# buaacyw/MeshAnything

Measured on NVIDIA H100. Metric: face-tokens/sec (350M, 800-face cap), higher is better.
Workload: dtype f16 weights/activations, f32 accumulate

## Files before the change

include/meshanything_b200.h:

```cpp
#ifndef MESHANYTHING_B200_H
#define MESHANYTHING_B200_H

#include <stddef.h>
#include <stdint.h>

#ifdef __cplusplus
extern "C" {
#endif

#define MA_ABI_VERSION 1
#define MA_MAX_LAYERS 32

#define MA_EPI_NONE 0
#define MA_EPI_RELU 1
#define MA_EPI_GELU 2
#define MA_LIN_SEG64 0x10
#define MA_LIN_SEG256 0x20

int ma_abi_version(void);
const char* ma_last_error(void);


int ma_linear_f16(const void* W, const void* bias, const void* x, int ldx, void* y, int ldy, int M, int N, int K,
                  int epilogue, void* stream);

int ma_layernorm(const float* x, const void* res16, const float* gamma, const float* beta, float eps, int M, int W,
                 float* out32, void* out16, void* stream);

size_t ma_attention_scratch_bytes(int M, int H, int max_keys);
int ma_attention_f16(const void* q, int ldq, const void* K, const void* V, long T, int H, const int* slots,
                     const int* nkeys, int max_keys, int M, float scale, void* out, int ldo, void* scratch,
                     void* stream);
int ma_attention_decode_f16(const void* qkv, int ldq, void* K, void* V, long T, const int* nkeys, int max_keys, int M,
                            float scale, void* out, int ldo, void* scratch, void* stream);


typedef struct {
  int n_layers, vocab, codebook, npos;
  const void* wqkv[MA_MAX_LAYERS];
  const void* bqkv[MA_MAX_LAYERS];
  const void* wo[MA_MAX_LAYERS];
  const void* bo[MA_MAX_LAYERS];
  const void* w1[MA_MAX_LAYERS];
  const void* b1[MA_MAX_LAYERS];
  const void* w2[MA_MAX_LAYERS];
  const void* b2[MA_MAX_LAYERS];
  const float* ln1g[MA_MAX_LAYERS];
  const float* ln1b[MA_MAX_LAYERS];
  const float* ln2g[MA_MAX_LAYERS];
  const float* ln2b[MA_MAX_LAYERS];
  const void* lm_head;
  const void* tok_table;
  const float* extra;
  const float* tok_pos;
  const float* cond;
  const float* pos;
} ma_decoder_weights;

typedef struct {
  int do_sample;
  int top_k;
  float top_p;
  uint64_t seed;
} ma_sampling;

int ma_sample_tokens(const void* logits, int B, int vocab, const ma_sampling* sampling, int32_t* out_tokens,
                     int32_t* out_support, void* stream);

size_t ma_kv_cache_bytes(int n_layers, int B, int tmax);
size_t ma_decoder_workspace_bytes(int B, int tmax);

int ma_decode_generate(const ma_decoder_weights* w, const float* prefix, int B, int tmax, int max_new,
                       const ma_sampling* sampling, int eos_id, int pad_id, void* kv, void* ws, int32_t* out_ids,
                       int32_t* out_lens, const int32_t* forced_ids, void* logits_out, int flags, void* stream);

int ma_decode_slots_init(int B, int tmax, int pad_id, void* ws, void* stream);
int ma_decode_slot_stream(int slot, int B, int tmax, int stream_id, void* ws, void* stream);
int ma_decode_slots_seek(int B, int tmax, int pos, int gen, int tok, void* ws, void* stream);
int ma_decode_slot_prefill(const ma_decoder_weights* w, const float* prefix, int slot, int B, int tmax, int max_new,
                           const ma_sampling* sampling, int eos_id, int pad_id, void* kv, void* ws, int32_t* out_ids,
                           void* stream);
int ma_decode_slots_step(const ma_decoder_weights* w, int B, int tmax, int max_new, int n_steps, int max_ctx,
                         const ma_sampling* sampling, int eos_id, int pad_id, void* kv, void* ws, int32_t* out_ids,
                         int flags, void* stream);
int ma_decode_slots_poll(int B, int tmax, void* ws, int32_t* finished_host, int32_t* lens_host, void* stream);

#define MA_GEN_NO_GRAPH 1
#define MA_GEN_NO_FAST 2
#define MA_GEN_NO_PDL 4
#define MA_GEN_NO_EARLY_EXIT 8
#define MA_GEN_NO_MEGA 16
#define MA_GEN_TC 64
#define MA_GEN_TRACE 32

int ma_decoder_debug(void* ws, int B, int tmax, int what, void* host_out, int nbytes);
void ma_mega_set_debug(unsigned long long timeout_ns, int fault);
int ma_decode_persistent_supported(void);


int ma_linear_tc_f16(const void* W, const void* bias, const void* x, int ldx, void* y, int ldy, int M, int N, int K,
                     int epilogue, void* stream);
size_t ma_linear_ws_scratch_bytes(void);
void ma_linear_ws_set_mode(int cluster);
int ma_linear_ws_f16(const void* W, const void* bias, const void* x, int ldx, void* y, int ldy, int M, int N, int K,
                     int epilogue, void* scratch, void* stream);
int ma_set_tensor_cores(int enable);
void ma_tensor_core_linear_counts(unsigned long long* on_tensor_cores, unsigned long long* canonical_fallback);

int ma_attention_tc_f16(const void* q, int ldq, const void* K, const void* Vt, long T, long Tpad, int H,
                        int rows_per_slot, int n_slots, int nkeys, float scale, void* out, int ldo, void* stream);
int ma_transpose_heads_f16(const void* src, int ld, int col0, int head_stride, int H, int n, long Tpad, int n_slots,
                           void* dst, void* stream);


typedef struct {
  const void* c_qkv_w;
  const void *c_proj_w, *c_proj_b;
  const float *ln1_g, *ln1_b, *ln2_g, *ln2_b;
  const void *fc_w, *fc_b;
  const void *proj_w, *proj_b;
} ma_miche_block;

typedef struct {
  const void *input_proj_w, *input_proj_b;
  const float* query;
  const void *cq_w, *ckv_w;
  const void *cproj_w, *cproj_b;
  const float *ln1_g, *ln1_b, *ln2_g, *ln2_b, *ln3_g, *ln3_b;
  const void *fc_w, *fc_b, *proj_w, *proj_b;
  ma_miche_block enc[8];
  const float *lnpost_g, *lnpost_b;
  const void *pre_kl_w, *pre_kl_b;
  const void *post_kl_w, *post_kl_b;
  ma_miche_block dec[16];
  const void *cond_head_w, *cond_head_b;
  const void *cond_w, *cond_b;
} ma_encoder_weights;

size_t ma_encoder_workspace_bytes(int B);

int ma_encoder_forward(const ma_encoder_weights* w, const void* pc_normal, int B, float* point_feature, float* prefix,
                       void* ws, void* stream);


typedef struct {
  const void *in_w, *in_b;
  const void *out_w, *out_b;
  const void *l1_w, *l1_b;
  const void *l2_w, *l2_b;
  const float *n1_g, *n1_b, *n2_g, *n2_b;
} ma_bert_layer;

typedef struct {
  int n_layers;
  ma_bert_layer layer[8];
  const float* pos_embedding;
  const float* point_pe;
  const float *ln_g, *ln_b, *pln_g, *pln_b;
  const void *cond_w, *cond_b, *cond_head_w, *cond_head_b;
  const void *down_w, *down_b;
  const void *coor_w, *coor_b;
  const float* codebook;
} ma_tokenizer_weights;

size_t ma_detokenize_workspace_bytes(int B, int F);

int ma_detokenize(const ma_tokenizer_weights* w, const int32_t* gen_ids, int max_new, int B, int F,
                  const float* point_feature, float* out_xyz, int32_t* ids_out, void* ws, void* stream);

size_t ma_sample_surface_workspace_bytes(int n_faces);
int ma_sample_surface(const float* vertices, const int32_t* faces, int n_faces, int n_samples, unsigned long long seed,
                      void* out_pc_normal, int32_t* out_face_idx, void* ws, void* stream);

unsigned long long ma_launch_count(void);

#ifdef __cplusplus
}
#endif
#endif
```

meshanything_b200/capi.py:

```python
from __future__ import annotations

import ctypes as C
import os
from typing import Optional

import torch

from . import build as _build

MA_MAX_LAYERS = 32
EPI_NONE, EPI_RELU, EPI_GELU = 0, 1, 2
LIN_SEG64, LIN_SEG256 = 0x10, 0x20
GEN_NO_GRAPH, GEN_NO_FAST, GEN_NO_PDL, GEN_NO_EARLY_EXIT, GEN_NO_MEGA, GEN_TRACE, GEN_TC = 1, 2, 4, 8, 16, 32, 64

_vp = C.c_void_p


class DecoderWeights(C.Structure):
    _fields_ = (
        [("n_layers", C.c_int), ("vocab", C.c_int), ("codebook", C.c_int), ("npos", C.c_int)]
        + [(n, _vp * MA_MAX_LAYERS) for n in ("wqkv", "bqkv", "wo", "bo", "w1", "b1", "w2", "b2",
                                              "ln1g", "ln1b", "ln2g", "ln2b")]
        + [(n, _vp) for n in ("lm_head", "tok_table", "extra", "tok_pos", "cond", "pos")]
    )


class Sampling(C.Structure):
    _fields_ = [("do_sample", C.c_int), ("top_k", C.c_int), ("top_p", C.c_float), ("seed", C.c_uint64)]


_lib = None

EXPORTS = [
    "ma_abi_version", "ma_last_error", "ma_launch_count", "ma_linear_f16", "ma_layernorm",
    "ma_attention_scratch_bytes", "ma_attention_f16", "ma_attention_decode_f16", "ma_kv_cache_bytes", "ma_decoder_workspace_bytes",
    "ma_decode_generate", "ma_decoder_debug", "ma_encoder_workspace_bytes", "ma_encoder_forward",
    "ma_detokenize_workspace_bytes", "ma_detokenize", "ma_linear_tc_f16", "ma_set_tensor_cores", "ma_sample_tokens",
    "ma_attention_tc_f16", "ma_transpose_heads_f16",
    "ma_decode_slots_init", "ma_decode_slot_prefill", "ma_decode_slots_step", "ma_decode_slots_poll",
    "ma_mega_set_debug", "ma_linear_ws_set_mode", "ma_decode_slots_seek", "ma_decode_slot_stream", "ma_linear_ws_scratch_bytes", "ma_linear_ws_f16",
    "ma_sample_surface_workspace_bytes", "ma_sample_surface", "ma_tensor_core_linear_counts", "ma_decode_persistent_supported",
]


def lib_path() -> str:
    return _build.LIB


def lib():
    global _lib
    if _lib is not None:
        return _lib
    path = _build.LIB
    dev_tree = os.path.isdir(os.path.join(os.path.dirname(os.path.dirname(os.path.abspath(__file__))), ".git"))
    stale = (os.path.exists(path) and dev_tree and _build.have_nvcc()
             and os.environ.get("MA_B200_NO_AUTOBUILD") != "1" and _build._stale())
    if not os.path.exists(path) or stale or (os.environ.get("MA_B200_REBUILD") == "1"):
        path = _build.build(force=True)
    L = C.CDLL(path)
    L.ma_abi_version.restype = C.c_int
    L.ma_last_error.restype = C.c_char_p
    L.ma_launch_count.restype = C.c_ulonglong
    L.ma_linear_f16.argtypes = [_vp, _vp, _vp, C.c_int, _vp, C.c_int, C.c_int, C.c_int, C.c_int, C.c_int, _vp]
    L.ma_layernorm.argtypes = [_vp, _vp, _vp, _vp, C.c_float, C.c_int, C.c_int, _vp, _vp, _vp]
    L.ma_attention_scratch_bytes.argtypes = [C.c_int, C.c_int, C.c_int]
    L.ma_attention_scratch_bytes.restype = C.c_size_t
    L.ma_attention_f16.argtypes = [_vp, C.c_int, _vp, _vp, C.c_long, C.c_int, _vp, _vp, C.c_int, C.c_int,
                                   C.c_float, _vp, C.c_int, _vp, _vp]
    L.ma_kv_cache_bytes.argtypes = [C.c_int, C.c_int, C.c_int]
    L.ma_kv_cache_bytes.restype = C.c_size_t
    L.ma_decoder_workspace_bytes.argtypes = [C.c_int, C.c_int]
    L.ma_decoder_workspace_bytes.restype = C.c_size_t
    L.ma_decode_generate.argtypes = [C.POINTER(DecoderWeights), _vp, C.c_int, C.c_int, C.c_int, C.POINTER(Sampling),
                                     C.c_int, C.c_int, _vp, _vp, _vp, _vp, _vp, _vp, C.c_int, _vp]
    L.ma_sample_tokens.argtypes = [_vp, C.c_int, C.c_int, C.POINTER(Sampling), _vp, _vp, _vp]
    L.ma_attention_decode_f16.argtypes = [_vp, C.c_int, _vp, _vp, C.c_long, _vp, C.c_int, C.c_int, C.c_float, _vp, C.c_int,
                                          _vp, _vp]
    L.ma_attention_tc_f16.argtypes = [_vp, C.c_int, _vp, _vp, C.c_long, C.c_long, C.c_int, C.c_int, C.c_int, C.c_int,
                                      C.c_float, _vp, C.c_int, _vp]
    L.ma_transpose_heads_f16.argtypes = [_vp, C.c_int, C.c_int, C.c_int, C.c_int, C.c_int, C.c_long, C.c_int, _vp, _vp]
    L.ma_decode_slots_init.argtypes = [C.c_int, C.c_int, C.c_int, _vp, _vp]
    L.ma_linear_ws_set_mode.argtypes = [C.c_int]
    L.ma_linear_ws_set_mode.restype = None
    L.ma_decode_slot_stream.argtypes = [C.c_int, C.c_int, C.c_int, C.c_int, _vp, _vp]
    L.ma_decode_slots_seek.argtypes = [C.c_int, C.c_int, C.c_int, C.c_int, C.c_int, _vp, _vp]
    L.ma_decode_slot_prefill.argtypes = [C.POINTER(DecoderWeights), _vp, C.c_int, C.c_int, C.c_int, C.c_int,
                                         C.POINTER(Sampling), C.c_int, C.c_int, _vp, _vp, _vp, _vp]
    L.ma_decode_slots_step.argtypes = [C.POINTER(DecoderWeights), C.c_int, C.c_int, C.c_int, C.c_int, C.c_int,
                                       C.POINTER(Sampling), C.c_int, C.c_int, _vp, _vp, _vp, C.c_int, _vp]
    L.ma_decode_slots_poll.argtypes = [C.c_int, C.c_int, _vp, _vp, _vp, _vp]
    L.ma_decoder_debug.argtypes = [_vp, C.c_int, C.c_int, C.c_int, _vp, C.c_int]
    L.ma_mega_set_debug.argtypes = [C.c_ulonglong, C.c_int]
    L.ma_mega_set_debug.restype = None
    L.ma_decode_persistent_supported.argtypes = []
    L.ma_decode_persistent_supported.restype = C.c_int
    L.ma_encoder_workspace_bytes.argtypes = [C.c_int]
    L.ma_encoder_workspace_bytes.restype = C.c_size_t
    L.ma_encoder_forward.argtypes = [_vp, _vp, C.c_int, _vp, _vp, _vp, _vp]
    L.ma_detokenize_workspace_bytes.argtypes = [C.c_int, C.c_int]
    L.ma_detokenize_workspace_bytes.restype = C.c_size_t
    L.ma_detokenize.argtypes = [_vp, _vp, C.c_int, C.c_int, C.c_int, _vp, _vp, _vp, _vp, _vp]
    L.ma_linear_ws_scratch_bytes.restype = C.c_size_t
    L.ma_linear_ws_f16.argtypes = [_vp, _vp, _vp, C.c_int, _vp, C.c_int, C.c_int, C.c_int, C.c_int, C.c_int, _vp, _vp]
    L.ma_sample_surface_workspace_bytes.argtypes = [C.c_int]
    L.ma_sample_surface_workspace_bytes.restype = C.c_size_t
    L.ma_sample_surface.argtypes = [_vp, _vp, C.c_int, C.c_int, C.c_ulonglong, _vp, _vp, _vp, _vp]
    L.ma_linear_tc_f16.argtypes = [_vp, _vp, _vp, C.c_int, _vp, C.c_int, C.c_int, C.c_int, C.c_int, C.c_int, _vp]
    L.ma_set_tensor_cores.argtypes = [C.c_int]
    L.ma_tensor_core_linear_counts.argtypes = [C.POINTER(C.c_ulonglong), C.POINTER(C.c_ulonglong)]
    L.ma_tensor_core_linear_counts.restype = None
    if L.ma_abi_version() != 1:
        raise RuntimeError("libmeshanything_b200.so: ABI version mismatch")
    _lib = L
    return L


def check(rc: int, what: str):
    if rc != 0:
        raise RuntimeError(f"{what} failed: {lib().ma_last_error().decode()}")


def ptr(t: Optional[torch.Tensor]):
    return None if t is None else C.c_void_p(t.data_ptr())


def stream_ptr() -> C.c_void_p:
    return C.c_void_p(torch.cuda.current_stream().cuda_stream)


def _need_cuda(*ts):
    for t in ts:
        if t is not None and not t.is_cuda:
            raise RuntimeError("meshanything_b200: tensors must live on a CUDA device (no CPU fallback)")



def linear_f16(w: torch.Tensor, bias: Optional[torch.Tensor], x: torch.Tensor, epilogue: int = EPI_NONE,
               out: Optional[torch.Tensor] = None) -> torch.Tensor:
    _need_cuda(w, bias, x)
    assert w.dtype == torch.float16 and x.dtype == torch.float16 and w.is_contiguous()
    assert x.dim() == 2 and x.stride(1) == 1
    M, K = x.shape
    N = w.shape[0]
    if out is None:
        out = torch.empty((M, N), dtype=torch.float16, device=x.device)
    check(lib().ma_linear_f16(ptr(w), ptr(bias), ptr(x), x.stride(0), ptr(out), out.stride(0), M, N, K, epilogue,
                              stream_ptr()), "ma_linear_f16")
    return out


def sample_surface(vertices: torch.Tensor, faces: torch.Tensor, n_samples: int, seed: int = 0,
                   want_index: bool = False):
    _need_cuda(vertices, faces)
    v = vertices.to(torch.float32).contiguous()
    f = faces.to(torch.int32).contiguous()
    F = f.shape[0]
    ws = torch.empty(lib().ma_sample_surface_workspace_bytes(F), dtype=torch.uint8, device=v.device)
    out = torch.empty((n_samples, 6), dtype=torch.float16, device=v.device)
    idx = torch.empty((n_samples,), dtype=torch.int32, device=v.device) if want_index else None
    check(lib().ma_sample_surface(ptr(v), ptr(f), F, n_samples, int(seed), ptr(out), ptr(idx), ptr(ws), stream_ptr()),
          "ma_sample_surface")
    return (out, idx) if want_index else out


def tensor_core_linear_counts():
    a, b = C.c_ulonglong(0), C.c_ulonglong(0)
    lib().ma_tensor_core_linear_counts(C.byref(a), C.byref(b))
    return a.value, b.value


_ws_scratch = {}


def linear_ws_f16(w: torch.Tensor, bias: Optional[torch.Tensor], x: torch.Tensor, epilogue: int = EPI_NONE) -> torch.Tensor:
    _need_cuda(w, bias, x)
    M, K = x.shape
    N = w.shape[0]
    scr = _ws_scratch.get(x.device)
    if scr is None:
        scr = _ws_scratch[x.device] = torch.zeros(lib().ma_linear_ws_scratch_bytes(), dtype=torch.uint8, device=x.device)
    out = torch.empty((M, N), dtype=torch.float16, device=x.device)
    check(lib().ma_linear_ws_f16(ptr(w), ptr(bias), ptr(x), x.stride(0), ptr(out), out.stride(0), M, N, K, epilogue,
                                 ptr(scr), stream_ptr()), "ma_linear_ws_f16")
    return out


def linear_tc_f16(w: torch.Tensor, bias: Optional[torch.Tensor], x: torch.Tensor, epilogue: int = EPI_NONE) -> torch.Tensor:
    _need_cuda(w, bias, x)
    M, K = x.shape
    N = w.shape[0]
    out = torch.empty((M, N), dtype=torch.float16, device=x.device)
    check(lib().ma_linear_tc_f16(ptr(w), ptr(bias), ptr(x), x.stride(0), ptr(out), out.stride(0), M, N, K, epilogue,
                                 stream_ptr()), "ma_linear_tc_f16")
    return out


def transpose_heads_f16(src: torch.Tensor, col0: int, head_stride: int, H: int, n: int, n_slots: int) -> torch.Tensor:
    _need_cuda(src)
    Tpad = (n + 127) // 128 * 128
    dst = torch.empty((n_slots, H, 64, Tpad), dtype=torch.float16, device=src.device)
    check(lib().ma_transpose_heads_f16(ptr(src), src.stride(0), col0, head_stride, H, n, Tpad, n_slots, ptr(dst),
                                       stream_ptr()), "ma_transpose_heads_f16")
    return dst


def attention_tc_f16(q: torch.Tensor, k: torch.Tensor, vt: torch.Tensor, nkeys: int, rows_per_slot: int,
                     scale: float = 0.125) -> torch.Tensor:
    _need_cuda(q, k, vt)
    S, H, T, _ = k.shape
    Tpad = vt.shape[3]
    assert q.is_contiguous() and k.is_contiguous() and vt.is_contiguous() and q.shape[0] == S * rows_per_slot
    out = torch.empty_like(q)
    check(lib().ma_attention_tc_f16(ptr(q), q.stride(0), ptr(k), ptr(vt), T, Tpad, H, rows_per_slot, S, nkeys,
                                    C.c_float(scale), ptr(out), out.stride(0), stream_ptr()), "ma_attention_tc_f16")
    return out


def sample_tokens(logits: torch.Tensor, do_sample: bool = True, top_k: int = 50, top_p: float = 0.95, seed: int = 0,
                  want_support: bool = False):
    _need_cuda(logits)
    assert logits.dtype == torch.float16 and logits.is_contiguous()
    B, vocab = logits.shape
    tok = torch.empty((B,), dtype=torch.int32, device=logits.device)
    sup = torch.empty((B, 256), dtype=torch.int32, device=logits.device) if want_support else None
    s = Sampling(int(do_sample), int(top_k), float(top_p), int(seed))
    check(lib().ma_sample_tokens(ptr(logits), B, vocab, C.byref(s), ptr(tok), ptr(sup), stream_ptr()),
          "ma_sample_tokens")
    return (tok, sup) if want_support else tok


def layernorm(x: Optional[torch.Tensor], res16: Optional[torch.Tensor], gamma: torch.Tensor, beta: torch.Tensor,
              eps: float = 1e-5, want32: bool = True, want16: bool = True):
    _need_cuda(x, res16, gamma, beta)
    src = x if x is not None else res16
    M, W = src.shape
    o32 = torch.empty((M, W), dtype=torch.float32, device=src.device) if want32 else None
    o16 = torch.empty((M, W), dtype=torch.float16, device=src.device) if want16 else None
    check(lib().ma_layernorm(ptr(x), ptr(res16), ptr(gamma), ptr(beta), eps, M, W, ptr(o32), ptr(o16), stream_ptr()),
          "ma_layernorm")
    return o32, o16


def attention_decode_f16(qkv: torch.Tensor, k: torch.Tensor, v: torch.Tensor, nkeys: torch.Tensor,
                         scale: float = 0.125) -> torch.Tensor:
    _need_cuda(qkv, k, v, nkeys)
    M = qkv.shape[0]
    assert qkv.shape[1] == 3072 and qkv.is_contiguous() and k.is_contiguous() and v.is_contiguous()
    assert k.shape[0] == M and k.shape[1] == 16 and k.shape[3] == 64
    T = k.shape[2]
    max_keys = int(nkeys.max().item())
    scratch = torch.zeros(lib().ma_attention_scratch_bytes(M, 16, max_keys), dtype=torch.uint8, device=qkv.device)
    out = torch.empty((M, 1024), dtype=torch.float16, device=qkv.device)
    check(lib().ma_attention_decode_f16(ptr(qkv), 3072, ptr(k), ptr(v), T, ptr(nkeys), max_keys, M, scale, ptr(out),
                                        1024, ptr(scratch), stream_ptr()), "ma_attention_decode_f16")
    return out


def attention_f16(q: torch.Tensor, k: torch.Tensor, v: torch.Tensor, nkeys: torch.Tensor,
                  slots: Optional[torch.Tensor] = None, scale: float = 0.125) -> torch.Tensor:
    _need_cuda(q, k, v, nkeys, slots)
    M, H, D = q.shape
    assert D == 64 and k.is_contiguous() and v.is_contiguous() and q.is_contiguous()
    T = k.shape[2]
    max_keys = int(nkeys.max().item())
    scratch = torch.zeros(lib().ma_attention_scratch_bytes(M, H, max_keys), dtype=torch.uint8, device=q.device)
    out = torch.empty((M, H, D), dtype=torch.float16, device=q.device)
    check(lib().ma_attention_f16(ptr(q), H * D, ptr(k), ptr(v), T, H, ptr(slots), ptr(nkeys), max_keys, M, scale,
                                 ptr(out), H * D, ptr(scratch), stream_ptr()), "ma_attention_f16")
    return out
```

meshanything_b200/csrc/api.cu:

```cuda
#include <stdarg.h>
#include <stdlib.h>
#include <stdio.h>
#include <string.h>

#include <atomic>
#include <map>
#include <mutex>
#include <vector>

#include "canon.cuh"
#include "internal.h"

namespace ma {

static thread_local char g_err[512] = "";
static std::atomic<unsigned long long> g_launches{0};

void set_error(const char* fmt, ...) {
  va_list ap;
  va_start(ap, fmt);
  vsnprintf(g_err, sizeof(g_err), fmt, ap);
  va_end(ap);
}
void count_launch(int n) { g_launches += (unsigned long long)n; }
bool check_launch(const char* what) {
  cudaError_t e = cudaPeekAtLastError();
  if (e != cudaSuccess) {
    set_error("%s: %s", what, cudaGetErrorString(e));
    cudaGetLastError();
    return false;
  }
  return true;
}

static inline size_t align_up(size_t x, size_t a = 256) { return (x + a - 1) / a * a; }

constexpr int PREFILL_SEQS = 8;

struct DecWs {
  float* hres;
  __half *x16, *qkv, *attn16, *y16, *f16, *logits, *lastx16;
  int* nkeys;
  SeqState s;
  int* all_done;
  void* attn_scratch;
  size_t attn_scratch_bytes;
  void* attn_scratch_pre;
  size_t attn_scratch_pre_bytes;
  void* fast;
  void* mega;
  void* tc_scratch;
  size_t total;
};

static DecWs carve(void* base, int B, int tmax, int vocab) {
  DecWs w;
  const size_t rows = (size_t)std::max(B, PREFIX * std::min(B, PREFILL_SEQS));
  size_t off = 0;
  auto take = [&](size_t bytes) {
    void* p = base ? (void*)((char*)base + off) : nullptr;
    off += align_up(bytes);
    return p;
  };
  w.hres = (float*)take(rows * HID * 4);
  w.x16 = (__half*)take(rows * HID * 2);
  w.qkv = (__half*)take(rows * QKV * 2);
  w.attn16 = (__half*)take(rows * HID * 2);
  w.y16 = (__half*)take(rows * HID * 2);
  w.f16 = (__half*)take(rows * FFN * 2);
  w.logits = (__half*)take((size_t)B * vocab * 2);
  w.lastx16 = (__half*)take((size_t)B * HID * 2);
  w.nkeys = (int*)take(rows * 4);
  w.s.pos = (int*)take((size_t)B * 4);
  w.s.gen = (int*)take((size_t)B * 4);
  w.s.tok = (int*)take((size_t)B * 4);
  w.s.finished = (int*)take((size_t)B * 4);
  w.s.lens = (int*)take((size_t)B * 4);
  w.s.sid = (int*)take((size_t)B * 4);
  w.all_done = (int*)take(256);
  w.attn_scratch_bytes = attention_scratch_bytes((int)B, NHEAD, tmax);
  w.attn_scratch = take(w.attn_scratch_bytes);
  w.attn_scratch_pre_bytes = attention_scratch_bytes(PREFIX * std::min(B, PREFILL_SEQS), NHEAD, PREFIX);
  w.attn_scratch_pre = take(w.attn_scratch_pre_bytes);
  w.fast = take(fast_workspace_bytes());
  w.mega = take(mega_workspace_bytes());
  w.tc_scratch = take(linear_ws_scratch_bytes());
  w.total = off;
  return w;
}

static inline __half* kv_layer(void* kv, int layer, int which, int B, long T) {
  return (__half*)kv + ((size_t)(layer * 2 + which) * B) * NHEAD * T * HD;
}

static const bool g_no_stream_attn = [] {
  const char* e = getenv("MA_B200_NO_STREAM_ATTN");
  return e && e[0] == '1';
}();

static const bool g_no_pdl = [] {
  const char* e = getenv("MA_B200_NO_PDL");
  return e && e[0] == '1';
}();

static int dec_linear(bool tc, const DecWs& ws, const void* W, const void* b, const __half* x, int ldx, __half* y, int ldy,
                      int M, int N, int K, int epi, cudaStream_t st, bool pdl = false) {
  if (tc) {
    const bool tiled_ok = M >= 64 && linear_tc_supported(M, N, K, ldx, ldy, x, W, y);
    const bool ws_ok = M <= 128 && linear_ws_supported(M, N, K, ldx, x, W);
    if (ws_ok && (linear_ws_mode() || !tiled_ok || K > 1024))
      return launch_linear_ws((const __half*)W, (const __half*)b, x, ldx, y, ldy, M, N, K, epi, ws.tc_scratch, st, pdl);
    if (tiled_ok) return launch_linear_tc((const __half*)W, (const __half*)b, x, ldx, y, ldy, M, N, K, epi, st);
  }
  return launch_linear((const __half*)W, (const __half*)b, x, ldx, y, ldy, M, N, K, epi, st);
}

static int run_layers(const ma_decoder_weights* w, const DecWs& ws, void* kv, int B, long T, int M, int rows_per_slot,
                      int slot0, int max_keys, cudaStream_t st, bool tc = false) {
  void* scratch = rows_per_slot > 1 ? ws.attn_scratch_pre : ws.attn_scratch;
  const bool pdl = tc && rows_per_slot == 1 && !g_no_pdl;
  for (int L = 0; L < w->n_layers; L++) {
    __half* kc = kv_layer(kv, L, 0, B, T) + (size_t)slot0 * NHEAD * T * HD;
    __half* vc = kv_layer(kv, L, 1, B, T) + (size_t)slot0 * NHEAD * T * HD;
    if (dec_linear(tc, ws, w->wqkv[L], w->bqkv[L], ws.x16, HID, ws.qkv, QKV, M, QKV, HID, MA_EPI_NONE, st, pdl)) return 1;
    if (rows_per_slot == 1 && !g_no_stream_attn) {
      if (launch_attention_decode(ws.qkv, QKV, kc, vc, T, ws.nkeys, max_keys, M, 0.125f, ws.attn16, HID, scratch, pdl,
                                  st)) return 1;
    } else {
      if (launch_kv_append(ws.qkv, M, rows_per_slot, ws.nkeys, kc, vc, T, st)) return 1;
      if (launch_attention(ws.qkv, QKV, kc, vc, T, NHEAD, rows_per_slot, nullptr, ws.nkeys, max_keys, M, 0.125f,
                           ws.attn16, HID, scratch, st)) return 1;
    }
    if (dec_linear(tc, ws, w->wo[L], w->bo[L], ws.attn16, HID, ws.y16, HID, M, HID, HID, MA_EPI_NONE, st, pdl)) return 1;
    if (launch_layernorm(ws.hres, ws.y16, w->ln1g[L], w->ln1b[L], MA_LN_EPS, M, HID, ws.hres, ws.x16, st, pdl)) return 1;
    if (dec_linear(tc, ws, w->w1[L], w->b1[L], ws.x16, HID, ws.f16, FFN, M, FFN, HID, MA_EPI_RELU, st, pdl)) return 1;
    if (dec_linear(tc, ws, w->w2[L], w->b2[L], ws.f16, FFN, ws.y16, HID, M, HID, FFN, MA_EPI_NONE, st, pdl)) return 1;
    if (launch_layernorm(ws.hres, ws.y16, w->ln2g[L], w->ln2b[L], MA_LN_EPS, M, HID, ws.hres, ws.x16, st, pdl)) return 1;
  }
  return 0;
}

struct GraphKey {
  const void *w, *kv, *ws, *out_ids, *forced, *logits_out;
  unsigned long long whash;
  int B, tmax, max_new, bucket, flags, do_sample, top_k, eos, pad, mode;
  float top_p;
  unsigned long long seed;
  bool operator<(const GraphKey& o) const { return memcmp(this, &o, sizeof(GraphKey)) < 0; }
};
static std::map<GraphKey, cudaGraphExec_t> g_graphs;
static std::map<cudaGraphExec_t, unsigned long long> g_graph_launches;
static cudaStream_t g_stream = nullptr;
static int* g_flag_host = nullptr;
static cudaEvent_t g_ev_in = nullptr, g_ev_out = nullptr, g_ev_flag = nullptr;

static int g_device = -1;
static std::mutex g_mu;

static int ensure_globals() {
  int dev = -1;
  if (cudaGetDevice(&dev) != cudaSuccess) {
    set_error("cudaGetDevice: %s", cudaGetErrorString(cudaGetLastError()));
    return 1;
  }
  if (g_device >= 0 && dev != g_device) {
    set_error("ma_decode_generate was first used on device %d; this process now runs on device %d "
              "(one process per GPU)", g_device, dev);
    return 1;
  }
  if (!g_stream) {
    if (cudaStreamCreateWithFlags(&g_stream, cudaStreamNonBlocking) != cudaSuccess ||
        cudaHostAlloc((void**)&g_flag_host, 64, cudaHostAllocDefault) != cudaSuccess ||
        cudaEventCreateWithFlags(&g_ev_in, cudaEventDisableTiming) != cudaSuccess ||
        cudaEventCreateWithFlags(&g_ev_out, cudaEventDisableTiming) != cudaSuccess ||
        cudaEventCreateWithFlags(&g_ev_flag, cudaEventDisableTiming) != cudaSuccess) {
      set_error("cannot create stream/events: %s", cudaGetErrorString(cudaGetLastError()));
      return 1;
    }
    g_device = dev;
  }
  return 0;
}


static int enqueue_batched_step(const ma_decoder_weights* w, const DecWs& ws, void* kv, int B, long T, int max_keys,
                                const SampleArgs& sa, cudaStream_t s, bool tc) {
  if (launch_embed_tokens(w, ws.s, B, ws.hres, ws.x16, ws.nkeys, s)) return 1;
  if (run_layers(w, ws, kv, B, T, B, 1, 0, max_keys, s, tc)) return 1;
  if (dec_linear(tc, ws, w->lm_head, nullptr, ws.x16, HID, ws.logits, w->vocab, B, w->vocab, HID, MA_EPI_NONE, s,
                 tc && !g_no_pdl)) return 1;
  return launch_sample(sa, s);
}

static inline bool use_tc(int B, int do_sample, int flags) { return B > 1 && (do_sample || (flags & MA_GEN_TC)); }

static unsigned long long weights_hash(const ma_decoder_weights* w) {
  unsigned long long h = 1469598103934665603ull;
  const unsigned char* pb = (const unsigned char*)w;
  for (size_t q = 0; q < sizeof(ma_decoder_weights); q++) h = (h ^ pb[q]) * 1099511628211ull;
  return h;
}

template <class F>
static int launch_cached_graph(const GraphKey& key, cudaStream_t st, F&& enqueue) {
  auto it = g_graphs.find(key);
  if (it == g_graphs.end()) {
    cudaGraph_t graph = nullptr;
    if (cudaStreamBeginCapture(st, cudaStreamCaptureModeThreadLocal) != cudaSuccess) {
      set_error("cudaStreamBeginCapture: %s", cudaGetErrorString(cudaGetLastError()));
      return 1;
    }
    const unsigned long long before = g_launches.load();
    int erc = enqueue(st);
    const unsigned long long per_step = g_launches.load() - before;
    cudaError_t ce = cudaStreamEndCapture(st, &graph);
    if (erc || ce != cudaSuccess || !graph) {
      if (!erc) set_error("cudaStreamEndCapture: %s", cudaGetErrorString(ce));
      cudaGetLastError();
      return 1;
    }
    cudaGraphExec_t exec = nullptr;
    ce = cudaGraphInstantiate(&exec, graph, 0);
    cudaGraphDestroy(graph);
    if (ce != cudaSuccess) {
      set_error("cudaGraphInstantiate: %s", cudaGetErrorString(ce));
      return 1;
    }
    if (g_graphs.size() > 64) {
      for (auto& kvp : g_graphs) cudaGraphExecDestroy(kvp.second);
      g_graphs.clear();
      g_graph_launches.clear();
    }
    it = g_graphs.emplace(key, exec).first;
    g_launches -= per_step;
    g_graph_launches[exec] = per_step;
  }
  if (cudaGraphLaunch(it->second, st) != cudaSuccess) {
    set_error("cudaGraphLaunch: %s", cudaGetErrorString(cudaGetLastError()));
    return 1;
  }
  g_launches += g_graph_launches[it->second];
  return 0;
}

static void fill_sample_args(SampleArgs& sa, const ma_decoder_weights* w, const DecWs& ws, int B, int max_new,
                             const ma_sampling* sampling, int eos_id, int pad_id, int32_t* out_ids) {
  memset(&sa, 0, sizeof(sa));
  sa.logits = ws.logits; sa.vocab = w->vocab; sa.B = B; sa.max_new = max_new; sa.eos_id = eos_id; sa.pad_id = pad_id;
  sa.do_sample = sampling ? sampling->do_sample : 0;
  sa.top_k = sampling ? sampling->top_k : 0;
  sa.top_p = sampling ? sampling->top_p : 1.0f;
  sa.seed = sampling ? sampling->seed : 0;
  sa.s = ws.s; sa.out_ids = out_ids;
}

static int check_decode_args(const char* who, const ma_decoder_weights* w, int B, int tmax, int max_new) {
  if (w->n_layers > MA_MAX_LAYERS || w->vocab > 8195 + 61) {
    set_error("%s: n_layers=%d / vocab=%d unsupported", who, w->n_layers, w->vocab);
    return 1;
  }
  if (B <= 0 || max_new <= 0 || PREFIX + max_new > tmax) {
    set_error("%s: B=%d, tmax=%d < 257 + max_new=%d", who, B, tmax, max_new);
    return 1;
  }
  if (PREFIX + max_new + 2 > w->npos) {
    set_error("%s: sequence of %d exceeds %d learned positions", who, PREFIX + max_new, w->npos - 2);
    return 1;
  }
  return 0;
}

}

using namespace ma;

extern "C" {

int ma_abi_version(void) { return MA_ABI_VERSION; }
const char* ma_last_error(void) { return g_err; }
unsigned long long ma_launch_count(void) { return g_launches.load(); }

int ma_linear_f16(const void* W, const void* bias, const void* x, int ldx, void* y, int ldy, int M, int N, int K,
                  int epilogue, void* stream) {
  return launch_linear((const __half*)W, (const __half*)bias, (const __half*)x, ldx, (__half*)y, ldy, M, N, K,
                       epilogue, (cudaStream_t)stream);
}

size_t ma_linear_ws_scratch_bytes(void) { return linear_ws_scratch_bytes(); }
void ma_linear_ws_set_mode(int cluster) { linear_ws_set_mode(cluster); }

int ma_linear_ws_f16(const void* W, const void* bias, const void* x, int ldx, void* y, int ldy, int M, int N, int K,
                     int epilogue, void* scratch, void* stream) {
  return launch_linear_ws((const __half*)W, (const __half*)bias, (const __half*)x, ldx, (__half*)y, ldy, M, N, K,
                          epilogue, scratch, (cudaStream_t)stream);
}

int ma_layernorm(const float* x, const void* res16, const float* gamma, const float* beta, float eps, int M, int W,
                 float* out32, void* out16, void* stream) {
  return launch_layernorm(x, (const __half*)res16, gamma, beta, eps, M, W, out32, (__half*)out16,
                          (cudaStream_t)stream);
}

size_t ma_attention_scratch_bytes(int M, int H, int max_keys) { return attention_scratch_bytes(M, H, max_keys); }

int ma_attention_f16(const void* q, int ldq, const void* K, const void* V, long T, int H, const int* slots,
                     const int* nkeys, int max_keys, int M, float scale, void* out, int ldo, void* scratch,
                     void* stream) {
  if (M > 65535) {
    set_error("ma_attention_f16: M=%d exceeds 65535 rows per call", M);
    return 1;
  }
  return launch_attention((const __half*)q, ldq, (const __half*)K, (const __half*)V, T, H, 1, slots, nkeys, max_keys, M,
                          scale, (__half*)out, ldo, scratch, (cudaStream_t)stream);
}

int ma_attention_decode_f16(const void* qkv, int ldq, void* K, void* V, long T, const int* nkeys, int max_keys, int M,
                            float scale, void* out, int ldo, void* scratch, void* stream) {
  if (!qkv || !K || !V || !nkeys || !out || !scratch || M < 1 || max_keys < 1 || max_keys > T || ldq < 3 * HID) {
    set_error("ma_attention_decode_f16: bad arguments (M=%d, max_keys=%d, T=%ld, ldq=%d)", M, max_keys, T, ldq);
    return 1;
  }
  return launch_attention_decode((const __half*)qkv, ldq, (__half*)K, (__half*)V, T, nkeys, max_keys, M, scale,
                                 (__half*)out, ldo, scratch, false, (cudaStream_t)stream);
}

int ma_sample_tokens(const void* logits, int B, int vocab, const ma_sampling* sampling, int32_t* out_tokens,
                     int32_t* out_support, void* stream) {
  if (!logits || !out_tokens || B < 1 || vocab < 1) {
    set_error("ma_sample_tokens: bad arguments");
    return 1;
  }
  SampleArgs sa;
  memset(&sa, 0, sizeof(sa));
  sa.logits = (const __half*)logits; sa.vocab = vocab; sa.B = B; sa.max_new = 1; sa.eos_id = -1; sa.pad_id = -1;
  sa.do_sample = sampling ? sampling->do_sample : 0;
  sa.top_k = sampling ? sampling->top_k : 0;
  sa.top_p = sampling ? sampling->top_p : 1.0f;
  sa.seed = sampling ? sampling->seed : 0;
  sa.first = 1; sa.token_out = out_tokens; sa.support_out = out_support;
  return launch_sample(sa, (cudaStream_t)stream);
}

size_t ma_kv_cache_bytes(int n_layers, int B, int tmax) {
  return (size_t)n_layers * 2 * B * NHEAD * (size_t)tmax * HD * sizeof(__half);
}

size_t ma_decoder_workspace_bytes(int B, int tmax) { return carve(nullptr, B, tmax, 8195 + 61).total; }

int ma_decode_generate(const ma_decoder_weights* w, const float* prefix, int B, int tmax, int max_new,
                       const ma_sampling* sampling, int eos_id, int pad_id, void* kv, void* ws_, int32_t* out_ids,
                       int32_t* out_lens, const int32_t* forced_ids, void* logits_out, int flags, void* stream) {
  if (!w || !prefix || !kv || !ws_ || !out_ids || B <= 0 || max_new <= 0) {
    set_error("ma_decode_generate: bad arguments");
    return 1;
  }
  if (check_decode_args("ma_decode_generate", w, B, tmax, max_new)) return 1;
  std::lock_guard<std::mutex> lock(g_mu);
  if (ensure_globals()) return 1;
  cudaStream_t user = (cudaStream_t)stream;
  cudaStream_t st = g_stream;
  cudaEventRecord(g_ev_in, user);
  cudaStreamWaitEvent(st, g_ev_in, 0);

  const long T = tmax;
  DecWs ws = carve(ws_, B, tmax, 8195 + 61);
  cudaMemsetAsync(ws.attn_scratch, 0, ws.attn_scratch_bytes, st);
  cudaMemsetAsync(ws.attn_scratch_pre, 0, ws.attn_scratch_pre_bytes, st);
  cudaMemsetAsync(ws.fast, 0, fast_workspace_bytes(), st);
  if (launch_fill_i32(out_ids, pad_id, (long)B * max_new, st)) return 1;

  SampleArgs sa;
  fill_sample_args(sa, w, ws, B, max_new, sampling, eos_id, pad_id, out_ids);
  sa.first = 1; sa.forced = forced_ids; sa.logits_out = (__half*)logits_out;
  sa.all_done = ws.all_done;

  const bool tc = use_tc(B, sa.do_sample, flags);
  if (tc) cudaMemsetAsync(ws.tc_scratch, 0, linear_ws_scratch_bytes(), st);
  const bool fast = (B == 1) && !(flags & MA_GEN_NO_FAST);
  bool mega = fast && !sa.do_sample && !(flags & MA_GEN_NO_MEGA) && mega_fits(tmax) && mega_supported();
  if (fast) sa.nkeys_next = fast_nkeys_ptr(ws.fast);
  if (mega && mega_prepare(w, ws.mega, st)) mega = false;

  for (int b0 = 0; b0 < B; b0 += PREFILL_SEQS) {
    const int nb = std::min(PREFILL_SEQS, B - b0), M = nb * PREFIX;
    if (launch_embed_prefix(w, prefix + (size_t)b0 * PREFIX * HID, nb, ws.hres, ws.x16, ws.nkeys, st)) return 1;
    if (run_layers(w, ws, kv, B, T, M, PREFIX, b0, PREFIX, st, tc)) return 1;
    if (launch_gather_rows(ws.x16, HID, PREFIX - 1, PREFIX, nb, ws.lastx16 + (size_t)b0 * HID, st)) return 1;
  }
  if (dec_linear(tc, ws, w->lm_head, nullptr, ws.lastx16, HID, ws.logits, w->vocab, B, w->vocab, HID, MA_EPI_NONE, st))
    return 1;
  if (launch_sample(sa, st)) return 1;
  sa.first = 0;
  sa.nkeys_next = nullptr;


  const bool use_graph = !(flags & MA_GEN_NO_GRAPH);
  const bool early = !(flags & MA_GEN_NO_EARLY_EXIT) && !forced_ids;
  const int CHECK_EVERY = 64;
  const unsigned long long whash = use_graph ? weights_hash(w) : 0;
  bool flag_pending = false;
  int rc = 0;
  if (mega) {
    const int MEGA_STEPS = 512;
    for (int i = 1; i < max_new && rc == 0; i += MEGA_STEPS) {
      rc = mega_enqueue(w, ws.s, tmax, (__half*)kv, ws.mega, sa, std::min(MEGA_STEPS, max_new - i), i - 1,
                        (flags & MA_GEN_TRACE) ? 1 : 0, st);
    }
  }
  for (int i = 1; i < max_new && rc == 0 && !mega; i++) {
    const int ctx = PREFIX + i;
    const int bucket = fast ? 0 : (ctx + 1023) / 1024;
    const int max_keys = fast ? tmax : std::min(tmax, bucket * 1024);
    auto enqueue = [&](cudaStream_t s) -> int {
      if (fast) return fast_step_enqueue(w, ws.s, tmax, (__half*)kv, ws.fast, sa, !(flags & MA_GEN_NO_PDL), s);
      return enqueue_batched_step(w, ws, kv, B, T, max_keys, sa, s, tc);
    };
    if (!use_graph) {
      rc = enqueue(st);
    } else {
      GraphKey key;
      memset(&key, 0, sizeof(key));
      key.w = w; key.kv = kv; key.ws = ws_; key.out_ids = out_ids; key.forced = forced_ids; key.logits_out = logits_out;
      key.B = B; key.tmax = tmax; key.max_new = max_new; key.bucket = bucket; key.flags = flags;
      key.do_sample = sa.do_sample; key.top_k = sa.top_k; key.eos = eos_id; key.pad = pad_id; key.top_p = sa.top_p;
      key.seed = sa.do_sample ? sa.seed : 0;
      key.whash = whash;
      if (launch_cached_graph(key, st, enqueue)) return 1;
    }
    if (early && (i % CHECK_EVERY) == 0) {
      if (flag_pending && cudaEventQuery(g_ev_flag) == cudaSuccess) {
        if (*g_flag_host == 1) break;
        flag_pending = false;
      }
      if (!flag_pending) {
        cudaMemcpyAsync(g_flag_host, ws.all_done, sizeof(int), cudaMemcpyDeviceToHost, st);
        cudaEventRecord(g_ev_flag, st);
        flag_pending = true;
      }
    }
  }
  if (rc) return rc;
  if (out_lens) cudaMemcpyAsync(out_lens, ws.s.lens, sizeof(int) * B, cudaMemcpyDeviceToDevice, st);
  cudaEventRecord(g_ev_out, st);
  cudaStreamWaitEvent(user, g_ev_out, 0);
  return check_launch("ma_decode_generate") ? 0 : 1;
}



static int slots_enter(void* stream, cudaStream_t* st) {
  if (ensure_globals()) return 1;
  cudaEventRecord(g_ev_in, (cudaStream_t)stream);
  cudaStreamWaitEvent(g_stream, g_ev_in, 0);
  *st = g_stream;
  return 0;
}
static int slots_leave(void* stream, const char* who) {
  cudaEventRecord(g_ev_out, g_stream);
  cudaStreamWaitEvent((cudaStream_t)stream, g_ev_out, 0);
  return check_launch(who) ? 0 : 1;
}

int ma_decode_slots_init(int B, int tmax, int pad_id, void* ws_, void* stream) {
  if (!ws_ || B <= 0 || tmax < PREFIX + 1) {
    set_error("ma_decode_slots_init: bad arguments");
    return 1;
  }
  std::lock_guard<std::mutex> lock(g_mu);
  cudaStream_t st;
  if (slots_enter(stream, &st)) return 1;
  DecWs ws = carve(ws_, B, tmax, 8195 + 61);
  cudaMemsetAsync(ws.attn_scratch, 0, ws.attn_scratch_bytes, st);
  cudaMemsetAsync(ws.attn_scratch_pre, 0, ws.attn_scratch_pre_bytes, st);
  cudaMemsetAsync(ws.tc_scratch, 0, linear_ws_scratch_bytes(), st);
  if (launch_fill_i32(ws.s.pos, PREFIX, B, st) || launch_fill_i32(ws.s.gen, 0, B, st) ||
      launch_fill_i32(ws.s.tok, pad_id, B, st) || launch_fill_i32(ws.s.finished, 1, B, st) ||
      launch_fill_i32(ws.s.lens, 0, B, st) || launch_fill_i32(ws.s.sid, 0, B, st)) return 1;
  return slots_leave(stream, "ma_decode_slots_init");
}

int ma_decode_slot_stream(int slot, int B, int tmax, int stream_id, void* ws_, void* stream) {
  if (!ws_ || slot < 0 || slot >= B) {
    set_error("ma_decode_slot_stream: bad arguments (slot %d of %d)", slot, B);
    return 1;
  }
  std::lock_guard<std::mutex> lock(g_mu);
  cudaStream_t st;
  if (slots_enter(stream, &st)) return 1;
  DecWs ws = carve(ws_, B, tmax, 8195 + 61);
  if (launch_fill_i32(ws.s.sid + slot, stream_id, 1, st)) return 1;
  return slots_leave(stream, "ma_decode_slot_stream");
}

int ma_decode_slots_seek(int B, int tmax, int pos, int gen, int tok, void* ws_, void* stream) {
  if (!ws_ || B <= 0 || pos < PREFIX || pos >= tmax || gen < 1) {
    set_error("ma_decode_slots_seek: bad arguments (pos %d of tmax %d)", pos, tmax);
    return 1;
  }
  std::lock_guard<std::mutex> lock(g_mu);
  cudaStream_t st;
  if (slots_enter(stream, &st)) return 1;
  DecWs ws = carve(ws_, B, tmax, 8195 + 61);
  if (launch_fill_i32(ws.s.pos, pos, B, st) || launch_fill_i32(ws.s.gen, gen, B, st) ||
      launch_fill_i32(ws.s.tok, tok, B, st) || launch_fill_i32(ws.s.finished, 0, B, st) ||
      launch_fill_i32(ws.s.lens, gen, B, st)) return 1;
  return slots_leave(stream, "ma_decode_slots_seek");
}

int ma_decode_slot_prefill(const ma_decoder_weights* w, const float* prefix, int slot, int B, int tmax, int max_new,
                           const ma_sampling* sampling, int eos_id, int pad_id, void* kv, void* ws_, int32_t* out_ids,
                           void* stream) {
  if (!w || !prefix || !kv || !ws_ || !out_ids || slot < 0 || slot >= B) {
    set_error("ma_decode_slot_prefill: bad arguments (slot %d of %d)", slot, B);
    return 1;
  }
  if (check_decode_args("ma_decode_slot_prefill", w, B, tmax, max_new)) return 1;
  std::lock_guard<std::mutex> lock(g_mu);
  cudaStream_t st;
  if (slots_enter(stream, &st)) return 1;
  const long T = tmax;
  DecWs ws = carve(ws_, B, tmax, 8195 + 61);
  if (launch_fill_i32(out_ids + (size_t)slot * max_new, pad_id, max_new, st)) return 1;
  if (launch_embed_prefix(w, prefix, 1, ws.hres, ws.x16, ws.nkeys, st)) return 1;
  const bool tc = use_tc(B, sampling ? sampling->do_sample : 0, 0);
  if (run_layers(w, ws, kv, B, T, PREFIX, PREFIX, slot, PREFIX, st, tc)) return 1;
  __half* last = ws.lastx16 + (size_t)slot * HID;
  if (launch_gather_rows(ws.x16, HID, PREFIX - 1, PREFIX, 1, last, st)) return 1;
  if (dec_linear(tc, ws, w->lm_head, nullptr, last, HID, ws.logits + (size_t)slot * w->vocab, w->vocab, 1, w->vocab, HID,
                 MA_EPI_NONE, st)) return 1;
  SampleArgs sa;
  fill_sample_args(sa, w, ws, B, max_new, sampling, eos_id, pad_id, out_ids);
  sa.first = 1; sa.row0 = slot; sa.nrows = 1; sa.slots = 1;
  if (launch_sample(sa, st)) return 1;
  return slots_leave(stream, "ma_decode_slot_prefill");
}

int ma_decode_slots_step(const ma_decoder_weights* w, int B, int tmax, int max_new, int n_steps, int max_ctx,
                         const ma_sampling* sampling, int eos_id, int pad_id, void* kv, void* ws_, int32_t* out_ids,
                         int flags, void* stream) {
  if (!w || !kv || !ws_ || !out_ids || n_steps < 0 || max_ctx < PREFIX + 1) {
    set_error("ma_decode_slots_step: bad arguments");
    return 1;
  }
  if (check_decode_args("ma_decode_slots_step", w, B, tmax, max_new)) return 1;
  std::lock_guard<std::mutex> lock(g_mu);
  cudaStream_t st;
  if (slots_enter(stream, &st)) return 1;
  const long T = tmax;
  DecWs ws = carve(ws_, B, tmax, 8195 + 61);
  SampleArgs sa;
  fill_sample_args(sa, w, ws, B, max_new, sampling, eos_id, pad_id, out_ids);
  sa.slots = 1;
  const bool use_graph = !(flags & MA_GEN_NO_GRAPH);
  const unsigned long long whash = use_graph ? weights_hash(w) : 0;
  for (int i = 0; i < n_steps; i++) {
    const int ctx = std::min(tmax, max_ctx + i);
    const int bucket = (ctx + 1023) / 1024;
    const int max_keys = std::min(tmax, bucket * 1024);
    auto enqueue = [&](cudaStream_t s) -> int {
      return enqueue_batched_step(w, ws, kv, B, T, max_keys, sa, s, use_tc(B, sa.do_sample, flags));
    };
    if (!use_graph) {
      if (enqueue(st)) return 1;
    } else {
      GraphKey key;
      memset(&key, 0, sizeof(key));
      key.w = w; key.kv = kv; key.ws = ws_; key.out_ids = out_ids;
      key.B = B; key.tmax = tmax; key.max_new = max_new; key.bucket = bucket; key.flags = flags; key.mode = 1;
      key.do_sample = sa.do_sample; key.top_k = sa.top_k; key.eos = eos_id; key.pad = pad_id; key.top_p = sa.top_p;
      key.seed = sa.do_sample ? sa.seed : 0;
      if (launch_cached_graph(key, st, enqueue)) return 1;
    }
  }
  return slots_leave(stream, "ma_decode_slots_step");
}

int ma_decode_slots_poll(int B, int tmax, void* ws_, int32_t* finished_host, int32_t* lens_host, void* stream) {
  if (!ws_ || !finished_host || !lens_host || B <= 0) {
    set_error("ma_decode_slots_poll: bad arguments");
    return 1;
  }
  std::lock_guard<std::mutex> lock(g_mu);
  cudaStream_t st;
  if (slots_enter(stream, &st)) return 1;
  DecWs ws = carve(ws_, B, tmax, 8195 + 61);
  cudaMemcpyAsync(finished_host, ws.s.finished, sizeof(int) * B, cudaMemcpyDeviceToHost, st);
  cudaMemcpyAsync(lens_host, ws.s.lens, sizeof(int) * B, cudaMemcpyDeviceToHost, st);
  if (cudaStreamSynchronize(st) != cudaSuccess) {
    set_error("ma_decode_slots_poll: %s", cudaGetErrorString(cudaGetLastError()));
    return 1;
  }
  return slots_leave(stream, "ma_decode_slots_poll");
}


void ma_mega_set_debug(unsigned long long timeout_ns, int fault) { mega_set_debug(timeout_ns, fault); }
int ma_decode_persistent_supported(void) { return mega_supported(); }

int ma_decoder_debug(void* ws_, int B, int tmax, int what, void* host_out, int nbytes) {
  DecWs ws = carve(ws_, B, tmax, 8195 + 61);
  cudaDeviceSynchronize();
  if (what == 0 && !mega_supported()) {
    memset(host_out, 0, (size_t)nbytes);
    return 0;
  }
  const char* src = (const char*)ws.mega + (what == 0 ? mega_error_flag_offset() : what == 1 ? mega_trace_offset() : mega_trace_cta_offset());
  return cudaMemcpy(host_out, src, (size_t)nbytes, cudaMemcpyDeviceToHost) == cudaSuccess ? 0 : 1;
}

}
```

meshanything_b200/csrc/decode_mega.cu:

```cuda
#include "canon.cuh"
#include "internal.h"

namespace ma {

constexpr int MG_THREADS = 512;
constexpr int MG_WARPS = 16;
constexpr int TEAM = 256;
constexpr int PARTF = 66;
constexpr int MAX_CHUNKS = 72;

struct MegaWs {
  uint2 qkv_w[QKV / 2];
  uint2 attn_w[HID / 2];
  uint2 ya_w[HID / 2];
  uint2 yb_w[HID / 2];
  uint2 f_w[FFN / 2];
  uint2 cand_w[256 * 2];
  int error;
  int pad_[3];
  unsigned long long trace[1280];
  unsigned long long trace_cta[160 * 8];
  ma_decoder_weights w;
  alignas(256) uint2 part_w[NHEAD * MAX_CHUNKS * PARTF];
  alignas(256) __half bias_cta[MA_MAX_LAYERS * 160 * 128];
};

constexpr int BIAS_QKV = 0, BIAS_OUT = 32, BIAS_FC1 = 48, BIAS_FC2 = 112;

struct MegaArgs {
  MegaWs* ws;
  SeqState s;
  __half* kv;
  long T;
  int n_steps, step_base, max_new, eos_id, pad_id;
  int rows_qkv, rows_out, rows_fc1, rows_fc2, rows_lm;
  int32_t* out_ids;
  const int32_t* forced;
  __half* logits_out;
  int* all_done;
  int* nkeys_next;
  int trace;
  int fault;
};

__device__ __forceinline__ unsigned long long gtimer() {
  unsigned long long t;
  asm volatile("mov.u64 %0, %globaltimer;" : "=l"(t));
  return t;
}

__device__ __forceinline__ void ll_store(uint2* p, uint32_t data, uint32_t ep) {
  asm volatile("st.volatile.global.v2.u32 [%0], {%1,%2};" ::"l"(p), "r"(data), "r"(ep) : "memory");
}
__device__ __forceinline__ uint4 ll_load2(const uint2* p) {
  uint4 v;
  asm volatile("ld.volatile.global.v4.u32 {%0,%1,%2,%3}, [%4];" : "=r"(v.x), "=r"(v.y), "=r"(v.z), "=r"(v.w) : "l"(p) : "memory");
  return v;
}
__device__ __forceinline__ uint2 ll_load1(const uint2* p) {
  uint2 v;
  asm volatile("ld.volatile.global.v2.u32 {%0,%1}, [%2];" : "=r"(v.x), "=r"(v.y) : "l"(p) : "memory");
  return v;
}
__constant__ unsigned c_spin_limit = 1u << 24;
#define SPIN_LIMIT c_spin_limit
__device__ __forceinline__ bool poll_giveup(int* err, unsigned& spins) {
  if ((++spins & 1023u) == 0) {
    if (*reinterpret_cast<volatile int*>(err)) return true;
    if (spins > SPIN_LIMIT) {
      atomicCAS(err, 0, 1 + (int)blockIdx.x);
      return true;
    }
  }
  return false;
}
__device__ __forceinline__ uint2 ll_wait2(const uint2* p, uint32_t ep, int* err) {
  uint4 v = ll_load2(p);
  unsigned spins = 0;
  while (v.y != ep || v.w != ep) {
    if (poll_giveup(err, spins)) break;
    v = ll_load2(p);
  }
  return make_uint2(v.x, v.z);
}
__device__ __forceinline__ uint32_t ll_wait1(const uint2* p, uint32_t ep, int* err) {
  uint2 v = ll_load1(p);
  unsigned spins = 0;
  while (v.y != ep) {
    if (poll_giveup(err, spins)) break;
    v = ll_load1(p);
  }
  return v.x;
}
template <int N>
__device__ __forceinline__ void ll_wait_units(const uint2* p, int stride, uint32_t ep, uint2* out, int* err) {
  uint4 v[N];
#pragma unroll
  for (int i = 0; i < N; i++) v[i] = ll_load2(p + 2 * i * stride);
  unsigned spins = 0;
  for (;;) {
    bool ok = true;
#pragma unroll
    for (int i = 0; i < N; i++) {
      if (v[i].y != ep || v[i].w != ep) {
        ok = false;
        v[i] = ll_load2(p + 2 * i * stride);
      }
    }
    if (ok) break;
    if (poll_giveup(err, spins)) break;
  }
#pragma unroll
  for (int i = 0; i < N; i++) out[i] = make_uint2(v[i].x, v[i].z);
}
__device__ __forceinline__ void store_x4(float* dst, uint2 d) {
  const __half2* hh = reinterpret_cast<const __half2*>(&d);
  const float2 p0 = __half22float2(hh[0]), p1 = __half22float2(hh[1]);
  *reinterpret_cast<float4*>(dst) = make_float4(p0.x, p0.y, p1.x, p1.y);
}
__device__ __forceinline__ void ll_gather(const uint2* src, int nhalf, uint32_t ep, __half* dst, int* err) {
  const int tid = threadIdx.x;
  if (nhalf == FFN) {
    uint2 d[2];
    ll_wait_units<2>(src + 2 * tid, MG_THREADS, ep, d, err);
    *reinterpret_cast<uint2*>(dst + 4 * tid) = d[0];
    *reinterpret_cast<uint2*>(dst + 4 * (tid + MG_THREADS)) = d[1];
  } else {
    for (int u = tid; u < nhalf / 4; u += MG_THREADS) {
      const uint2 d = ll_wait2(src + 2 * u, ep, err);
      *reinterpret_cast<uint2*>(dst + 4 * u) = d;
    }
  }
}

struct alignas(128) MegaSmem {
  uint64_t bar[4];
  uint64_t lnbar[2];
  uint64_t bbar[2];
  alignas(16) float ln1[2 * HID];
  alignas(16) float ln2[2 * HID];
  alignas(16) __half bias[2][128];
  ma_decoder_weights wtab;
  int errflag;
  float red[2][8];
  float wmax[2][8];
  float ared[2][8][65];
  float bval[MG_WARPS];
  int bidx[MG_WARPS];
  float cstage[2 * 2 * MAX_CHUNKS];
  alignas(16) __half stage16[64];
  alignas(16) float hres[HID];
  alignas(16) __half xs[FFN];
};

__device__ __forceinline__ uint4 ldcg16(const void* p) { return __ldcg(reinterpret_cast<const uint4*>(p)); }
__device__ __forceinline__ void fence_proxy_async() { asm volatile("fence.proxy.async.shared::cta;" ::: "memory"); }

__device__ __forceinline__ void layernorm_1024(float* v, const float* gamma, const float* beta, float (*red)[8], int tid) {
  if (tid >= 256) return;
  const int warp = tid >> 5, lane = tid & 31;
  const float inv = __fdiv_rn(1.0f, 1024.0f);
  float p = fadd(fadd(v[0], v[1]), fadd(v[2], v[3]));
  p = warp_sum(p);
  if (lane == 0) red[0][warp] = p;
  asm volatile("bar.sync 3, 256;" ::: "memory");
  const float mean = fmul(warp_tree(red[0], 8), inv);
  const float d0 = fsub(v[0], mean), d1 = fsub(v[1], mean), d2 = fsub(v[2], mean), d3 = fsub(v[3], mean);
  float q = fadd(fadd(fmul(d0, d0), fmul(d1, d1)), fadd(fmul(d2, d2), fmul(d3, d3)));
  q = warp_sum(q);
  if (lane == 0) red[1][warp] = q;
  asm volatile("bar.sync 3, 256;" ::: "memory");
  const float var = fmul(warp_tree(red[1], 8), inv);
  const float rstd = __fdiv_rn(1.0f, __fsqrt_rn(fadd(var, MA_LN_EPS)));
  const float4 g = *reinterpret_cast<const float4*>(gamma + 4 * tid);
  const float4 b = *reinterpret_cast<const float4*>(beta + 4 * tid);
  v[0] = ffma(fmul(d0, rstd), g.x, b.x);
  v[1] = ffma(fmul(d1, rstd), g.y, b.y);
  v[2] = ffma(fmul(d2, rstd), g.z, b.z);
  v[3] = ffma(fmul(d3, rstd), g.w, b.w);
}

__device__ __forceinline__ void team_sync(int team) { asm volatile("bar.sync %0, %1;" ::"r"(1 + team), "r"(TEAM) : "memory"); }

__device__ __forceinline__ void load_x8(const float* p, float* xf) {
  const float4 a = *reinterpret_cast<const float4*>(p), b = *reinterpret_cast<const float4*>(p + 4);
  xf[0] = a.x; xf[1] = a.y; xf[2] = a.z; xf[3] = a.w; xf[4] = b.x; xf[5] = b.y; xf[6] = b.z; xf[7] = b.w;
}

template <int K, bool RELU>
__device__ __forceinline__ void gemv_stage(const __half* sw, int nrows, const __half* bias, const __half* xs, int warp,
                                           int lane, __half* stage) {
  constexpr int G = K / 256;
  if (warp >= nrows) return;
  const __half* w[4];
  bool has[4];
#pragma unroll
  for (int i = 0; i < 4; i++) {
    const int r = warp + MG_WARPS * i;
    has[i] = r < nrows;
    w[i] = sw + (size_t)(has[i] ? r : warp) * K + 8 * lane;
  }
  float acc[4] = {0.0f, 0.0f, 0.0f, 0.0f};
  if (!has[1]) {
#pragma unroll 4
    for (int g = 0; g < G; g++) {
      float xf[8], f[8];
      unpack8(*reinterpret_cast<const uint4*>(xs + 256 * g + 8 * lane), xf);
      unpack8(*reinterpret_cast<const uint4*>(w[0] + 256 * g), f);
#pragma unroll
      for (int j = 0; j < 8; j++) acc[0] = ffma(f[j], xf[j], acc[0]);
    }
  } else if (!has[2]) {
#pragma unroll 4
    for (int g = 0; g < G; g++) {
      float xf[8], f0[8], f1[8];
      unpack8(*reinterpret_cast<const uint4*>(xs + 256 * g + 8 * lane), xf);
      unpack8(*reinterpret_cast<const uint4*>(w[0] + 256 * g), f0);
      unpack8(*reinterpret_cast<const uint4*>(w[1] + 256 * g), f1);
#pragma unroll
      for (int j = 0; j < 8; j++) {
        acc[0] = ffma(f0[j], xf[j], acc[0]);
        acc[1] = ffma(f1[j], xf[j], acc[1]);
      }
    }
  } else {
#pragma unroll 2
    for (int g = 0; g < G; g++) {
      float xf[8], f[4][8];
      unpack8(*reinterpret_cast<const uint4*>(xs + 256 * g + 8 * lane), xf);
#pragma unroll
      for (int i = 0; i < 4; i++) unpack8(*reinterpret_cast<const uint4*>(w[i] + 256 * g), f[i]);
#pragma unroll
      for (int j = 0; j < 8; j++) {
#pragma unroll
        for (int i = 0; i < 4; i++) acc[i] = ffma(f[i][j], xf[j], acc[i]);
      }
    }
  }
#pragma unroll
  for (int i = 0; i < 4; i++) {
    if (i == 0 || has[1]) acc[i] = warp_sum(acc[i]);
  }
  if (lane == 0) {
#pragma unroll
    for (int i = 0; i < 4; i++) {
      if (has[i]) {
        const int r = warp + MG_WARPS * i;
        __half h = __float2half_rn(fadd(acc[i], bias ? __half2float(bias[r]) : 0.0f));
        if (RELU && __half2float(h) < 0.0f) h = __float2half_rn(0.0f);
        stage[r] = h;
      }
    }
  }
}

__device__ __forceinline__ uint32_t pack2(__half a, __half b) {
  return (uint32_t)__half_as_ushort(a) | ((uint32_t)__half_as_ushort(b) << 16);
}

__device__ __forceinline__ void refill(__half* dst, const void* W, int row0, int nrows, int K, uint64_t* bar) {
  fence_proxy_async();
  if (nrows > 0) {
    const uint32_t bytes = (uint32_t)nrows * K * 2;
    mbar_expect_tx(bar, bytes);
    bulk_g2s(dst, reinterpret_cast<const __half*>(W) + (size_t)row0 * K, bytes, bar);
  } else {
    mbar_expect_tx(bar, 0);
  }
}

__device__ __forceinline__ void fill_ln(float* dst, const float* g, const float* b, uint64_t* bar) {
  fence_proxy_async();
  mbar_expect_tx(bar, 2u * HID * 4);
  bulk_g2s(dst, g, HID * 4, bar);
  bulk_g2s(dst + HID, b, HID * 4, bar);
}
__device__ __forceinline__ void fill_bias(__half* dst, const __half* src, uint64_t* bar) {
  fence_proxy_async();
  mbar_expect_tx(bar, 256);
  bulk_g2s(dst, src, 256, bar);
}

__global__ void __launch_bounds__(MG_THREADS, 1) decode_mega_kernel(MegaArgs a) {
  extern __shared__ __align__(128) unsigned char smem_raw[];
  MegaSmem& sm = *reinterpret_cast<MegaSmem*>(smem_raw);
  __half* bufD = reinterpret_cast<__half*>(smem_raw + sizeof(MegaSmem));
  __half* bufC = bufD + (size_t)a.rows_qkv * HID;
  __half* bufA = bufC + (size_t)a.rows_out * HID;
  __half* bufB = bufA + (size_t)a.rows_fc1 * HID;
  const int tid = threadIdx.x, warp = tid >> 5, lane = tid & 31;
  const int team = warp >> 3, wt = warp & 7, tl = tid & (TEAM - 1);
  const int grp = lane >> 3, li = lane & 7;
  MegaWs* ws = a.ws;
  {
    const uint32_t* src = reinterpret_cast<const uint32_t*>(&ws->w);
    uint32_t* dst = reinterpret_cast<uint32_t*>(&sm.wtab);
    for (int i = tid; i < (int)(sizeof(ma_decoder_weights) / 4); i += MG_THREADS) dst[i] = src[i];
  }
  if (tid == 0) sm.errflag = *reinterpret_cast<volatile int*>(&ws->error);
  __syncthreads();
  if (sm.errflag) return;
  const ma_decoder_weights& W = sm.wtab;
  const int NL = W.n_layers;
  const long T = a.T;
  int* err = &ws->error;

  const int cta = blockIdx.x, ncta = gridDim.x;
  const int row0_qkv = cta * a.rows_qkv, n_qkv = max(0, min(a.rows_qkv, QKV - row0_qkv));
  const int row0_out = cta * a.rows_out, n_out = max(0, min(a.rows_out, HID - row0_out));
  const int row0_fc1 = cta * a.rows_fc1, n_fc1 = max(0, min(a.rows_fc1, FFN - row0_fc1));
  const int row0_fc2 = cta * a.rows_fc2, n_fc2 = max(0, min(a.rows_fc2, HID - row0_fc2));
  const int row0_lm = cta * a.rows_lm, n_lm = max(0, min(a.rows_lm, W.vocab - row0_lm));
  const int lmD = min(n_lm, a.rows_qkv), lmC = max(0, min(n_lm, a.rows_qkv + a.rows_out) - a.rows_qkv),
            lmA = max(0, n_lm - a.rows_qkv - a.rows_out);

  uint32_t parD = 0, parC = 0, parA = 0, parB = 0, parL1 = 0, parL2 = 0, parB0 = 0, parB1 = 0;
  int lc = 0;
  if (tid == 0) {
    for (int i = 0; i < 4; i++) mbar_init(&sm.bar[i], 1);
    for (int i = 0; i < 2; i++) { mbar_init(&sm.lnbar[i], 1); mbar_init(&sm.bbar[i], 1); }
    mbar_fence_init();
    fill_ln(sm.ln1, W.ln1g[0], W.ln1b[0], &sm.lnbar[0]);
    fill_ln(sm.ln2, W.ln2g[0], W.ln2b[0], &sm.lnbar[1]);
    fill_bias(sm.bias[0], ws->bias_cta + ((size_t)0 * 160 + cta) * 128, &sm.bbar[0]);
    fill_bias(sm.bias[1], ws->bias_cta + ((size_t)(NL > 1 ? 1 : 0) * 160 + cta) * 128, &sm.bbar[1]);
    refill(bufD, W.wqkv[0], row0_qkv, n_qkv, HID, &sm.bar[0]);
    refill(bufC, W.wo[0], row0_out, n_out, HID, &sm.bar[1]);
    refill(bufA, W.w1[0], row0_fc1, n_fc1, HID, &sm.bar[2]);
    refill(bufB, W.w2[0], row0_fc2, n_fc2, FFN, &sm.bar[3]);
  }
  __syncthreads();

  int pos = a.s.pos[0], gen = a.s.gen[0], tok = a.s.tok[0], fin = a.s.finished[0];
  unsigned long long* tr = (a.trace && cta == 0 && tid == 0) ? ws->trace : nullptr;
  int tri = 0;
#define STAMP() do { if (tr && tri < 1270) tr[tri++] = gtimer(); } while (0)
#define CSTAMP(k) do { if (a.trace && tid == 0 && step == 1 && L == NL / 2) ws->trace_cta[cta * 8 + (k)] = gtimer(); } while (0)

  auto publish_x = [&](const float* v, bool keep_hres) {
    if (tid < 256) {
      if (keep_hres) *reinterpret_cast<float4*>(sm.hres + 4 * tid) = make_float4(v[0], v[1], v[2], v[3]);
      __half2 h0 = __floats2half2_rn(v[0], v[1]), h1 = __floats2half2_rn(v[2], v[3]);
      uint2 u;
      u.x = *reinterpret_cast<uint32_t*>(&h0);
      u.y = *reinterpret_cast<uint32_t*>(&h1);
      *reinterpret_cast<uint2*>(sm.xs + 4 * tid) = u;
    }
  };
  auto residual_in = [&](const uint2* words, uint32_t ep, float* v) {
    if (tid < 256) {
      const float4 hv = *reinterpret_cast<const float4*>(sm.hres + 4 * tid);
      const uint2 d = ll_wait2(words + 2 * tid, ep, err);
      const __half2* hh = reinterpret_cast<const __half2*>(&d);
      const float2 p0 = __half22float2(hh[0]), p1 = __half22float2(hh[1]);
      v[0] = fadd(hv.x, p0.x); v[1] = fadd(hv.y, p0.y); v[2] = fadd(hv.z, p1.x); v[3] = fadd(hv.w, p1.y);
    } else {
      v[0] = v[1] = v[2] = v[3] = 0.0f;
    }
  };

  for (int step = 0; step < a.n_steps; step++) {
    if (gen >= a.max_new || fin) break;
    const int nkeys = pos + 1;
    const int nch = (nkeys + MA_ATTN_CHUNK - 1) / MA_ATTN_CHUNK;
    const int nitems = nch * NHEAD;
    const uint32_t ep0 = (uint32_t)(a.step_base + step) * (uint32_t)NL + 1u;
    STAMP();

    for (int L = 0; L < NL; L++) {
      const uint32_t ep = ep0 + (uint32_t)L;
      const int bsel = lc & 1;
      const __half* lb = sm.bias[bsel];
      __half* kc = a.kv + ((size_t)(L * 2 + 0)) * NHEAD * T * HD;
      __half* vc = a.kv + ((size_t)(L * 2 + 1)) * NHEAD * T * HD;

      uint4 kreg[8], vreg[8];
      int item = team * ncta + (ncta - 1 - cta);
      if (item < nitems) {
        const int c = item >> 4, h = item & 15;
        const long base = ((long)h * T + (long)c * MA_ATTN_CHUNK) * HD;
#pragma unroll
        for (int rho = 0; rho < 8; rho++) {
          const int r = 32 * rho + 4 * wt + grp;
          if (c * MA_ATTN_CHUNK + r < pos) {
            kreg[rho] = ldcg16(kc + base + (long)r * HD + 8 * li);
            vreg[rho] = ldcg16(vc + base + (long)r * HD + 8 * li);
          }
        }
      }

      {
        float v[4] = {0.0f, 0.0f, 0.0f, 0.0f};
        if (L == 0) {
          if (tid < 256) {
            float4 X;
            int fidx;
            if (tok < 3) {
              X = *reinterpret_cast<const float4*>(W.extra + (long)tok * HID + 4 * tid);
              fidx = tok;
            } else {
              const uint2 u = *reinterpret_cast<const uint2*>(reinterpret_cast<const __half*>(W.tok_table) +
                                                              (long)(tok - 3) * HID + 4 * tid);
              const __half2* hh = reinterpret_cast<const __half2*>(&u);
              const float2 p0 = __half22float2(hh[0]), p1 = __half22float2(hh[1]);
              X = make_float4(p0.x, p0.y, p1.x, p1.y);
              int r = (gen - 2) % 9;
              if (r < 0) r += 9;
              fidx = r + 3;
            }
            const float4 F = *reinterpret_cast<const float4*>(W.tok_pos + (long)fidx * HID + 4 * tid);
            const float4 C = *reinterpret_cast<const float4*>(W.cond + HID + 4 * tid);
            const float4 P = *reinterpret_cast<const float4*>(W.pos + (long)(pos + 2) * HID + 4 * tid);
            v[0] = fadd(fadd(fadd(X.x, F.x), C.x), P.x);
            v[1] = fadd(fadd(fadd(X.y, F.y), C.y), P.y);
            v[2] = fadd(fadd(fadd(X.z, F.z), C.z), P.z);
            v[3] = fadd(fadd(fadd(X.w, F.w), C.w), P.w);
          }
        } else {
          residual_in(ws->yb_w, ep - 1, v);
          mbar_wait(&sm.lnbar[1], parL2);
          parL2 ^= 1;
          layernorm_1024(v, sm.ln2, sm.ln2 + HID, sm.red, tid);
        }
        publish_x(v, true);
      }
      __syncthreads();
      if (L > 0 && tid == 0) fill_ln(sm.ln2, W.ln2g[L], W.ln2b[L], &sm.lnbar[1]);
      STAMP();
      CSTAMP(0);
      mbar_wait(&sm.bbar[bsel], bsel ? parB1 : parB0);
      if (bsel) parB1 ^= 1; else parB0 ^= 1;
      mbar_wait(&sm.bar[0], parD);
      parD ^= 1;
      STAMP();
      gemv_stage<HID, false>(bufD, n_qkv, lb + BIAS_QKV, sm.xs, warp, lane, sm.stage16);
      STAMP();
      __syncthreads();
      STAMP();
      if (tid < (n_qkv >> 1)) {
        const int n = row0_qkv + 2 * tid;
        const uint32_t d = *reinterpret_cast<const uint32_t*>(sm.stage16 + 2 * tid);
        ll_store(ws->qkv_w + (n >> 1), d, ep);
        if (n >= HID) {
          const int e = (n - HID) & (HID - 1), head = e >> 6, dd = e & 63;
          __half* c = (n < 2 * HID) ? kc : vc;
          *reinterpret_cast<uint32_t*>(c + ((long)head * T + pos) * HD + dd) = d;
        }
      }
      if (tid == 0) {
        if (L + 1 < NL) refill(bufD, W.wqkv[L + 1], row0_qkv, n_qkv, HID, &sm.bar[0]);
        else refill(bufD, W.lm_head, row0_lm, lmD, HID, &sm.bar[0]);
      }
      STAMP();
      CSTAMP(1);

      for (int it = 0; item < nitems; item += 2 * ncta, it++) {
        const int c = item >> 4, h = item & 15;
        const int len = min(MA_ATTN_CHUNK, nkeys - c * MA_ATTN_CHUNK);
        const long base = ((long)h * T + (long)c * MA_ATTN_CHUNK) * HD;
        const int cur = pos - c * MA_ATTN_CHUNK;
#pragma unroll
        for (int rho = 0; rho < 8; rho++) {
          const int r = 32 * rho + 4 * wt + grp;
          if (r < len && it > 0 && r != cur) {
            kreg[rho] = ldcg16(kc + base + (long)r * HD + 8 * li);
            vreg[rho] = ldcg16(vc + base + (long)r * HD + 8 * li);
          }
        }
        float qf[8];
        {
          uint2 d[2];
          ll_wait_units<2>(ws->qkv_w + (h * HD + 8 * li) / 2, 1, ep, d, err);
          unpack8(make_uint4(d[0].x, d[0].y, d[1].x, d[1].y), qf);
        }
        if (cur >= 0 && cur < MA_ATTN_CHUNK) {
          const int rho_c = cur >> 5, gl_c = cur & 31;
          if (4 * wt + grp == gl_c) {
            uint2 kk[2], vv[2];
            ll_wait_units<2>(ws->qkv_w + (HID + h * HD + 8 * li) / 2, 1, ep, kk, err);
            ll_wait_units<2>(ws->qkv_w + (2 * HID + h * HD + 8 * li) / 2, 1, ep, vv, err);
            const uint2 k0 = kk[0], k1 = kk[1], v0 = vv[0], v1 = vv[1];
#pragma unroll
            for (int rho = 0; rho < 8; rho++)
              if (rho == rho_c) {
                kreg[rho] = make_uint4(k0.x, k0.y, k1.x, k1.y);
                vreg[rho] = make_uint4(v0.x, v0.y, v1.x, v1.y);
              }
          }
        }
        float pr[8];
#pragma unroll
        for (int rho = 0; rho < 8; rho++) {
          float kf[8];
          unpack8(kreg[rho], kf);
          float p = 0.0f;
#pragma unroll
          for (int j = 0; j < 8; j++) p = ffma(qf[j], kf[j], p);
          pr[rho] = p;
        }
#pragma unroll
        for (int sft = 4; sft >= 1; sft >>= 1) {
          const bool up = (li & sft) != 0;
#pragma unroll
          for (int i = 0; i < sft; i++) {
            const float mine = up ? pr[i + sft] : pr[i];
            const float other = up ? pr[i] : pr[i + sft];
            pr[i] = fadd(mine, __shfl_xor_sync(0xffffffffu, other, sft));
          }
        }
        const float s_own = fmul(pr[0], 0.125f);
        const bool own_valid = 32 * li + 4 * wt + grp < len;
        float lmax = own_valid ? s_own : -INFINITY;
        lmax = warp_max(lmax);
        team_sync(team);
        if (lane == 0) sm.wmax[team][wt] = lmax;
        team_sync(team);
        float cmax = sm.wmax[team][0];
#pragma unroll
        for (int w2 = 1; w2 < 8; w2++) cmax = fmaxf(cmax, sm.wmax[team][w2]);
        const float e_own = own_valid ? ma_exp(fsub(s_own, cmax)) : 0.0f;
        float l = 0.0f, o[8];
#pragma unroll
        for (int j = 0; j < 8; j++) o[j] = 0.0f;
#pragma unroll
        for (int rho = 0; rho < 8; rho++) {
          const int r = 32 * rho + 4 * wt + grp;
          const float e = __shfl_sync(0xffffffffu, e_own, (lane & 24) | rho);
          if (r < len) {
            l = fadd(l, e);
            const float pf = __half2float(__float2half_rn(e));
            float vf[8];
            unpack8(vreg[rho], vf);
#pragma unroll
            for (int j = 0; j < 8; j++) o[j] = ffma(pf, vf[j], o[j]);
          }
        }
        l = fadd(l, __shfl_xor_sync(0xffffffffu, l, 16));
        l = fadd(l, __shfl_xor_sync(0xffffffffu, l, 8));
#pragma unroll
        for (int j = 0; j < 8; j++) {
          o[j] = fadd(o[j], __shfl_xor_sync(0xffffffffu, o[j], 16));
          o[j] = fadd(o[j], __shfl_xor_sync(0xffffffffu, o[j], 8));
        }
        if (grp == 0) {
#pragma unroll
          for (int j = 0; j < 8; j++) sm.ared[team][wt][8 * li + j] = o[j];
          if (li == 0) sm.ared[team][wt][64] = l;
        }
        team_sync(team);
        if (tl < 65) {
          float x[8];
#pragma unroll
          for (int w2 = 0; w2 < 8; w2++) x[w2] = sm.ared[team][w2][tl];
          const float rsum = fadd(fadd(fadd(x[0], x[1]), fadd(x[2], x[3])), fadd(fadd(x[4], x[5]), fadd(x[6], x[7])));
          uint2* part = ws->part_w + ((long)h * MAX_CHUNKS + c) * PARTF;
          ll_store(part + (tl < 64 ? tl : 65), __float_as_uint(rsum), ep);
          if (tl == 64) ll_store(part + 64, __float_as_uint(cmax), ep);
        }
      }
      if (tl == 0) {
        const int Ln = (L + 1 < NL) ? L + 1 : 0;
        const __half* kn = a.kv + ((size_t)(Ln * 2 + 0)) * NHEAD * T * HD;
        const __half* vn = a.kv + ((size_t)(Ln * 2 + 1)) * NHEAD * T * HD;
        for (int it2 = team * ncta + (ncta - 1 - cta); it2 < nitems; it2 += 2 * ncta) {
          const int c2 = it2 >> 4, h2 = it2 & 15;
          const uint32_t bytes = (uint32_t)min(MA_ATTN_CHUNK, nkeys - c2 * MA_ATTN_CHUNK) * HD * 2;
          const long off = ((long)h2 * T + (long)c2 * MA_ATTN_CHUNK) * HD;
          asm volatile("cp.async.bulk.prefetch.L2.global [%0], %1;" ::"l"(kn + off), "r"(bytes) : "memory");
          asm volatile("cp.async.bulk.prefetch.L2.global [%0], %1;" ::"l"(vn + off), "r"(bytes) : "memory");
        }
      }
      STAMP();
      CSTAMP(2);
      if (team == 0 && ncta - 1 - cta < NHEAD) {
        const int h = ncta - 1 - cta;
        const uint2* part = ws->part_w + (long)h * MAX_CHUNKS * PARTF;
        float* ost = reinterpret_cast<float*>(sm.xs);
        float* wgt = sm.cstage + team * 2 * MAX_CHUNKS;
        float* mst = wgt + MAX_CHUNKS;
        const bool single = nch <= 31;
        team_sync(team);
        if (!single) {
          for (int i = tl; i < nch; i += TEAM) mst[i] = __uint_as_float(ll_wait1(part + (long)i * PARTF + 64, ep, err));
          team_sync(team);
          float M = -INFINITY;
          for (int cc = 0; cc < nch; cc++) M = fmaxf(M, mst[cc]);
          for (int i = tl; i < nch; i += TEAM) wgt[i] = ma_exp(fsub(mst[i], M));
        }
        float Lsum = 0.0f, O = 0.0f;
        for (int c0 = 0; c0 < nch; c0 += 31) {
          const int nb = min(31, nch - c0), nw = nb * PARTF;
          {
            uint2 w[8];
#pragma unroll
            for (int k = 0; k < 8; k++) {
              const int i = tl + TEAM * k;
              if (i < nw) w[k] = ll_load1(part + (long)c0 * PARTF + i);
            }
            unsigned spins = 0;
            for (;;) {
              bool ok = true;
#pragma unroll
              for (int k = 0; k < 8; k++) {
                const int i = tl + TEAM * k;
                if (i < nw && w[k].y != ep) {
                  ok = false;
                  w[k] = ll_load1(part + (long)c0 * PARTF + i);
                }
              }
              if (ok) break;
              if (poll_giveup(err, spins)) break;
            }
#pragma unroll
            for (int k = 0; k < 8; k++) {
              const int i = tl + TEAM * k;
              if (i < nw) ost[i] = __uint_as_float(w[k].x);
            }
          }
          team_sync(team);
          if (single) {
            float M = -INFINITY;
            for (int cc = 0; cc < nch; cc++) M = fmaxf(M, ost[cc * PARTF + 64]);
            for (int i = tl; i < nch; i += TEAM) wgt[i] = ma_exp(fsub(ost[i * PARTF + 64], M));
            team_sync(team);
          }
          if (tl < 64) {
            for (int cc = 0; cc < nb; cc++) {
              const float wc = wgt[c0 + cc];
              Lsum = ffma(ost[cc * PARTF + 65], wc, Lsum);
              O = ffma(ost[cc * PARTF + tl], wc, O);
            }
          }
          team_sync(team);
        }
        if (tl < 64) {
          const __half r = __float2half_rn(__fdiv_rn(O, Lsum));
          const __half r2 = __shfl_down_sync(0xffffffffu, r, 1);
          if ((tl & 1) == 0) ll_store(ws->attn_w + (h * HD + tl) / 2, pack2(r, r2), ep);
        }
      }
      STAMP();
      CSTAMP(3);

      if (n_out > 0) {
        ll_gather(ws->attn_w, HID, ep, sm.xs, err);
        __syncthreads();
        mbar_wait(&sm.bar[1], parC);
        gemv_stage<HID, false>(bufC, n_out, lb + BIAS_OUT, sm.xs, warp, lane, sm.stage16);
        __syncthreads();
        const bool withhold = a.fault && cta == a.fault - 1 && a.step_base + step >= 2;
        if (tid < (n_out >> 1) && !withhold)
          ll_store(ws->ya_w + ((row0_out + 2 * tid) >> 1), *reinterpret_cast<const uint32_t*>(sm.stage16 + 2 * tid), ep);
      } else {
        __syncthreads();
        mbar_wait(&sm.bar[1], parC);
      }
      parC ^= 1;
      if (tid == 0) {
        if (L + 1 < NL) refill(bufC, W.wo[L + 1], row0_out, n_out, HID, &sm.bar[1]);
        else refill(bufC, W.lm_head, row0_lm + a.rows_qkv, lmC, HID, &sm.bar[1]);
      }
      STAMP();
      CSTAMP(4);

      {
        float v[4];
        residual_in(ws->ya_w, ep, v);
        mbar_wait(&sm.lnbar[0], parL1);
        parL1 ^= 1;
        layernorm_1024(v, sm.ln1, sm.ln1 + HID, sm.red, tid);
        publish_x(v, true);
      }
      __syncthreads();
      if (tid == 0) fill_ln(sm.ln1, W.ln1g[(L + 1) % NL], W.ln1b[(L + 1) % NL], &sm.lnbar[0]);
      mbar_wait(&sm.bar[2], parA);
      parA ^= 1;
      gemv_stage<HID, true>(bufA, n_fc1, lb + BIAS_FC1, sm.xs, warp, lane, sm.stage16);
      __syncthreads();
      if (tid < (n_fc1 >> 1))
        ll_store(ws->f_w + ((row0_fc1 + 2 * tid) >> 1), *reinterpret_cast<const uint32_t*>(sm.stage16 + 2 * tid), ep);
      if (tid == 0) {
        if (L + 1 < NL) refill(bufA, W.w1[L + 1], row0_fc1, n_fc1, HID, &sm.bar[2]);
        else refill(bufA, W.lm_head, row0_lm + a.rows_qkv + a.rows_out, lmA, HID, &sm.bar[2]);
      }
      STAMP();
      CSTAMP(5);

      if (n_fc2 > 0) {
        ll_gather(ws->f_w, FFN, ep, sm.xs, err);
        __syncthreads();
        mbar_wait(&sm.bar[3], parB);
        gemv_stage<FFN, false>(bufB, n_fc2, lb + BIAS_FC2, sm.xs, warp, lane, sm.stage16);
        __syncthreads();
        if (tid < (n_fc2 >> 1))
          ll_store(ws->yb_w + ((row0_fc2 + 2 * tid) >> 1), *reinterpret_cast<const uint32_t*>(sm.stage16 + 2 * tid), ep);
      } else {
        __syncthreads();
        mbar_wait(&sm.bar[3], parB);
      }
      parB ^= 1;
      if (tid == 0) {
        refill(bufB, W.w2[(L + 1 < NL) ? L + 1 : 0], row0_fc2, n_fc2, FFN, &sm.bar[3]);
        fill_bias(sm.bias[bsel], ws->bias_cta + ((size_t)((L + 2) % NL) * 160 + cta) * 128, &sm.bbar[bsel]);
      }
      lc++;
      STAMP();
      CSTAMP(6);
    }

    const uint32_t epc = (uint32_t)(a.step_base + step) + 1u;
    {
      float v[4];
      residual_in(ws->yb_w, ep0 + (uint32_t)NL - 1u, v);
      mbar_wait(&sm.lnbar[1], parL2);
      parL2 ^= 1;
      layernorm_1024(v, sm.ln2, sm.ln2 + HID, sm.red, tid);
      publish_x(v, false);
    }
    __syncthreads();
    if (tid == 0) fill_ln(sm.ln2, W.ln2g[0], W.ln2b[0], &sm.lnbar[1]);
    mbar_wait(&sm.bar[0], parD);
    mbar_wait(&sm.bar[1], parC);
    mbar_wait(&sm.bar[2], parA);
    parD ^= 1; parC ^= 1; parA ^= 1;
    gemv_stage<HID, false>(bufD, n_lm, nullptr, sm.xs, warp, lane, sm.stage16);
    __syncthreads();
    float bestv = -INFINITY;
    int besti = 0x7fffffff;
    if (tid < n_lm) {
      const __half hv = sm.stage16[tid];
      if (a.logits_out) a.logits_out[(long)gen * W.vocab + row0_lm + tid] = hv;
      bestv = __half2float(hv);
      besti = row0_lm + tid;
    }
    if (warp < 2) {
#pragma unroll
      for (int o = 16; o > 0; o >>= 1) {
        const float ov = __shfl_xor_sync(0xffffffffu, bestv, o);
        const int oi = __shfl_xor_sync(0xffffffffu, besti, o);
        if (ov > bestv || (ov == bestv && oi < besti)) { bestv = ov; besti = oi; }
      }
      if (lane == 0) { sm.bval[warp] = bestv; sm.bidx[warp] = besti; }
    }
    __syncthreads();
    if (tid == 0) {
      float bv = sm.bval[0];
      int bi = sm.bidx[0];
      if (sm.bval[1] > bv || (sm.bval[1] == bv && sm.bidx[1] < bi)) { bv = sm.bval[1]; bi = sm.bidx[1]; }
      __threadfence();
      ll_store(ws->cand_w + 2 * cta, __float_as_uint(bv), epc);
      ll_store(ws->cand_w + 2 * cta + 1, (uint32_t)bi, epc);
      refill(bufD, W.wqkv[0], row0_qkv, n_qkv, HID, &sm.bar[0]);
      refill(bufC, W.wo[0], row0_out, n_out, HID, &sm.bar[1]);
      refill(bufA, W.w1[0], row0_fc1, n_fc1, HID, &sm.bar[2]);
    }
    {
      float bv = -INFINITY;
      int bi = 0x7fffffff;
      if (tid < ncta) {
        const uint2 d = ll_wait2(ws->cand_w + 2 * tid, epc, err);
        bv = __uint_as_float(d.x);
        bi = (int)d.y;
      }
#pragma unroll
      for (int o = 16; o > 0; o >>= 1) {
        const float ov = __shfl_xor_sync(0xffffffffu, bv, o);
        const int oi = __shfl_xor_sync(0xffffffffu, bi, o);
        if (ov > bv || (ov == bv && oi < bi)) { bv = ov; bi = oi; }
      }
      __syncthreads();
      if (lane == 0) { sm.bval[warp] = bv; sm.bidx[warp] = bi; }
      if (tid == 0) sm.errflag = *reinterpret_cast<volatile int*>(&ws->error);
      __syncthreads();
      bv = sm.bval[0];
      bi = sm.bidx[0];
      for (int w2 = 1; w2 < MG_WARPS; w2++)
        if (sm.bval[w2] > bv || (sm.bval[w2] == bv && sm.bidx[w2] < bi)) { bv = sm.bval[w2]; bi = sm.bidx[w2]; }
      if (sm.errflag) break;
      int ntok = bi;
      if (a.forced) ntok = a.forced[gen];
      if (fin) ntok = a.pad_id;
      if (cta == 0 && tid == 0) {
        if (gen < a.max_new) a.out_ids[gen] = ntok;
        if (!fin) a.s.lens[0] = gen + 1;
      }
      if (!fin && ntok == a.eos_id) fin = 1;
      tok = ntok;
      gen += 1;
      pos += 1;
      __syncthreads();
    }
    STAMP();
  }

  mbar_wait(&sm.bar[0], parD);
  mbar_wait(&sm.bar[1], parC);
  mbar_wait(&sm.bar[2], parA);
  mbar_wait(&sm.bar[3], parB);
  mbar_wait(&sm.lnbar[0], parL1);
  mbar_wait(&sm.lnbar[1], parL2);
  mbar_wait(&sm.bbar[0], parB0);
  mbar_wait(&sm.bbar[1], parB1);
  if (cta == 0 && tid == 0) {
    const int e = *reinterpret_cast<volatile int*>(&ws->error);
    a.s.pos[0] = pos; a.s.gen[0] = gen; a.s.tok[0] = tok; a.s.finished[0] = e ? 1 : fin;
    if (e) a.s.lens[0] = -1;
    if (a.nkeys_next) *a.nkeys_next = pos + 1;
    if (a.all_done) *a.all_done = e ? 1 : fin;
  }
}

static int g_mega_sms = 0;
size_t mega_workspace_bytes() { return sizeof(MegaWs) + 256; }

static int mega_sms() {
  if (!g_mega_sms) {
    int dev = 0;
    cudaGetDevice(&dev);
    cudaDeviceGetAttribute(&g_mega_sms, cudaDevAttrMultiProcessorCount, dev);
    if (g_mega_sms <= 0 || g_mega_sms > 160) g_mega_sms = 132;
  }
  return g_mega_sms;
}
static inline int mega_rpc(int N) { return (((N + mega_sms() - 1) / mega_sms()) + 1) & ~1; }

__global__ void mega_pack_bias_kernel(MegaWs* ws, int rq, int ro, int r1, int r2) {
  const int L = blockIdx.y, cta = blockIdx.x, t = threadIdx.x;
  const ma_decoder_weights& W = ws->w;
  __half v = __float2half_rn(0.0f);
  if (t < BIAS_OUT) {
    const int n = cta * rq + t;
    if (t < rq && n < QKV) v = reinterpret_cast<const __half*>(W.bqkv[L])[n];
  } else if (t < BIAS_FC1) {
    const int i = t - BIAS_OUT, n = cta * ro + i;
    if (i < ro && n < HID) v = reinterpret_cast<const __half*>(W.bo[L])[n];
  } else if (t < BIAS_FC2) {
    const int i = t - BIAS_FC1, n = cta * r1 + i;
    if (i < r1 && n < FFN) v = reinterpret_cast<const __half*>(W.b1[L])[n];
  } else {
    const int i = t - BIAS_FC2, n = cta * r2 + i;
    if (i < r2 && n < HID) v = reinterpret_cast<const __half*>(W.b2[L])[n];
  }
  ws->bias_cta[((size_t)L * 160 + cta) * 128 + t] = v;
}

int mega_prepare(const ma_decoder_weights* w, void* mega_ws, cudaStream_t st) {
  MegaWs* ws = reinterpret_cast<MegaWs*>(mega_ws);
  if (cudaMemsetAsync(ws, 0, offsetof(MegaWs, bias_cta), st) != cudaSuccess) return 1;
  if (cudaMemcpyAsync(&ws->w, w, sizeof(ma_decoder_weights), cudaMemcpyHostToDevice, st) != cudaSuccess) return 1;
  const int rq = mega_rpc(QKV), ro = mega_rpc(HID), r1 = mega_rpc(FFN), r2 = mega_rpc(HID);
  if (rq > 32 || ro > 16 || r1 > 64 || r2 > 16) {
    set_error("mega: rows per CTA out of range");
    return 1;
  }
  mega_pack_bias_kernel<<<dim3(160, w->n_layers), 128, 0, st>>>(ws, rq, ro, r1, r2);
  count_launch();
  return check_launch("mega_pack_bias_kernel") ? 0 : 1;
}

static int g_mega_fault = 0;
void mega_set_debug(unsigned long long timeout_ns, int fault) {
  if (timeout_ns) {
    const unsigned long long polls = timeout_ns / 400ull + 2048ull;
    const unsigned v = polls > 0xffffffffull ? 0xffffffffu : (unsigned)polls;
    cudaMemcpyToSymbol(c_spin_limit, &v, sizeof(v));
  }
  g_mega_fault = fault;
}
bool mega_fits(int tmax) { return tmax <= MAX_CHUNKS * MA_ATTN_CHUNK; }
int mega_supported() {
  static int ok = -1;
  if (ok < 0) {
    const int sms = mega_sms(), r1 = mega_rpc(FFN), ro = mega_rpc(HID);
    const int grid = (FFN + r1 - 1) / r1;
    ok = (grid <= sms && grid >= NHEAD && grid - NHEAD >= (HID + ro - 1) / ro && mega_rpc(QKV) <= 32 && ro <= 16 && r1 <= 64) ? 1 : 0;
    if (!ok) set_error("mega: unsupported SM count %d", sms);
  }
  return ok;
}
int mega_error_flag_offset() { return (int)offsetof(MegaWs, error); }
int mega_trace_offset() { return (int)offsetof(MegaWs, trace); }
int mega_trace_cta_offset() { return (int)offsetof(MegaWs, trace_cta); }

int mega_enqueue(const ma_decoder_weights* w, SeqState s, int tmax, __half* kv, void* mega_ws, const SampleArgs& sa,
                 int n_steps, int step_base, int trace, cudaStream_t st) {
  if (tmax > MAX_CHUNKS * MA_ATTN_CHUNK) {
    set_error("mega: tmax=%d exceeds %d keys", tmax, MAX_CHUNKS * MA_ATTN_CHUNK);
    return 1;
  }
  const int sms = mega_sms();
  auto rpc = [&](int N) { return mega_rpc(N); };
  MegaArgs a;
  memset(&a, 0, sizeof(a));
  a.ws = reinterpret_cast<MegaWs*>(mega_ws);
  a.s = s;
  a.kv = kv;
  a.T = tmax;
  a.n_steps = n_steps;
  a.step_base = step_base;
  a.max_new = sa.max_new; a.eos_id = sa.eos_id; a.pad_id = sa.pad_id;
  a.rows_qkv = rpc(QKV); a.rows_out = rpc(HID); a.rows_fc1 = rpc(FFN); a.rows_fc2 = rpc(HID); a.rows_lm = rpc(w->vocab);
  a.out_ids = sa.out_ids; a.forced = sa.forced; a.logits_out = sa.logits_out; a.all_done = sa.all_done;
  a.nkeys_next = sa.nkeys_next;
  a.trace = trace;
  a.fault = g_mega_fault;
  if (a.rows_lm > a.rows_qkv + a.rows_out + a.rows_fc1 || a.rows_lm > 64 || a.rows_fc1 > 64) {
    set_error("mega: rows per CTA out of range (lm %d, fc1 %d)", a.rows_lm, a.rows_fc1);
    return 1;
  }
  const int grid = (FFN + a.rows_fc1 - 1) / a.rows_fc1;
  if (grid > sms || (w->vocab + a.rows_lm - 1) / a.rows_lm != grid || grid < NHEAD) {
    set_error("mega: unsupported SM count %d (grid %d)", sms, grid);
    return 1;
  }
  if (grid - NHEAD < (HID + a.rows_out - 1) / a.rows_out) {
    set_error("mega: the last %d CTAs must not own out_proj rows (grid %d)", NHEAD, grid);
    return 1;
  }
  const size_t smem = sizeof(MegaSmem) + ((size_t)(a.rows_qkv + a.rows_out + a.rows_fc1) * HID + (size_t)a.rows_fc2 * FFN) * 2;
  static size_t attr_set = 0;
  if (smem > attr_set) {
    if (cudaFuncSetAttribute(decode_mega_kernel, cudaFuncAttributeMaxDynamicSharedMemorySize, (int)smem) != cudaSuccess) {
      set_error("mega: cannot get %zu bytes of shared memory", smem);
      cudaGetLastError();
      return 1;
    }
    attr_set = smem;
  }
  cudaLaunchConfig_t cfg = {};
  cfg.gridDim = dim3(grid);
  cfg.blockDim = dim3(MG_THREADS);
  cfg.dynamicSmemBytes = smem;
  cfg.stream = st;
  cudaLaunchAttribute at[1];
  at[0].id = cudaLaunchAttributeCooperative;
  at[0].val.cooperative = 1;
  cfg.attrs = at;
  cfg.numAttrs = 1;
  cudaLaunchKernelEx(&cfg, decode_mega_kernel, a);
  count_launch();
  return check_launch("decode_mega_kernel") ? 0 : 1;
}

}
```

meshanything_b200/csrc/internal.h:

```cpp
#pragma once
#include <cuda_fp16.h>
#include <cuda_runtime.h>
#include <stdint.h>

#include "../../include/meshanything_b200.h"

namespace ma {

constexpr int HID = 1024;
constexpr int NHEAD = 16;
constexpr int HD = 64;
constexpr int FFN = 4096;
constexpr int PREFIX = 257;
constexpr int QKV = 3 * HID;

struct SeqState {
  int* pos;
  int* gen;
  int* tok;
  int* finished;
  int* lens;
  int* sid;
};

void set_error(const char* fmt, ...);
void count_launch(int n = 1);
bool check_launch(const char* what);

int launch_linear(const __half* W, const __half* bias, const __half* x, int ldx, __half* y, int ldy, int M, int N,
                  int K, int epi, cudaStream_t st);

bool attention_tc_supported(int ldq, int ldo, long T, long Tpad, int nkeys, const void* q, const void* K, const void* Vt,
                            const void* out);
int launch_attention_tc(const __half* q, int ldq, const __half* K, const __half* Vt, long T, long Tpad, int H,
                        int rows_per_slot, int n_slots, int nkeys, float scale, __half* out, int ldo, cudaStream_t st);
int launch_scatter_heads_t(const __half* src, int ld, int col0, int head_stride, int H, int n, long Tpad, int n_slots,
                           __half* dst, cudaStream_t st);

bool linear_tc_supported(int M, int N, int K, int ldx, int ldy, const void* x, const void* W, const void* y);
int launch_linear_tc(const __half* W, const __half* bias, const __half* x, int ldx, __half* y, int ldy, int M, int N,
                     int K, int epi, cudaStream_t st);

size_t linear_ws_scratch_bytes();
void linear_ws_set_mode(int cluster);
int linear_ws_mode();
bool linear_ws_supported(int M, int N, int K, int ldx, const void* x, const void* W);
int launch_linear_ws(const __half* W, const __half* bias, const __half* x, int ldx, __half* y, int ldy, int M, int N,
                     int K, int epi, void* scratch, cudaStream_t st, bool pdl = false);

size_t attention_scratch_bytes(int M, int H, int max_keys);
int launch_attention_decode(const __half* qkv, int ldq, __half* K, __half* V, long T, const int* nkeys, int max_keys,
                            int M, float scale, __half* out, int ldo, void* scratch, bool pdl, cudaStream_t st);
int launch_attention(const __half* q, int ldq, const __half* K, const __half* V, long T, int H, int rows_per_slot,
                     const int* slots, const int* nkeys, int max_keys, int M, float scale, __half* out, int ldo,
                     void* scratch, cudaStream_t st);

int launch_layernorm(const float* x, const __half* res16, const float* gamma, const float* beta, float eps, int M,
                     int W, float* out32, __half* out16, cudaStream_t st, bool pdl = false);
int launch_embed_prefix(const ma_decoder_weights* w, const float* prefix, int B, float* hres, __half* x16, int* nkeys,
                        cudaStream_t st);
int launch_embed_tokens(const ma_decoder_weights* w, SeqState s, int B, float* hres, __half* x16, int* nkeys,
                        cudaStream_t st);
int launch_kv_append(const __half* qkv, int M, int rows_per_slot, const int* nkeys, __half* kc, __half* vc, long T,
                     cudaStream_t st);
int launch_gather_rows(const __half* src, int ld, int row0, int stride, int B, __half* dst, cudaStream_t st);
struct SampleArgs {
  const __half* logits;
  int vocab, B, max_new, eos_id, pad_id;
  int do_sample, top_k;
  float top_p;
  unsigned long long seed;
  SeqState s;
  int first;
  int32_t* out_ids;
  const int32_t* forced;
  __half* logits_out;
  int* all_done;
  int* nkeys_next;
  int32_t* support_out;
  int32_t* token_out;
  int row0, nrows;
  int slots;
};
int launch_sample(const SampleArgs& a, cudaStream_t st);
int launch_fill_i32(int32_t* p, int v, long n, cudaStream_t st);

int* fast_nkeys_ptr(void* fast_ws);
size_t fast_workspace_bytes();
int fast_step_enqueue(const ma_decoder_weights* w, SeqState s, int tmax, __half* kv, void* fast_ws,
                      const SampleArgs& sa, bool pdl, cudaStream_t st);


size_t mega_workspace_bytes();
int mega_prepare(const ma_decoder_weights* w, void* mega_ws, cudaStream_t st);
int mega_enqueue(const ma_decoder_weights* w, SeqState s, int tmax, __half* kv, void* mega_ws, const SampleArgs& sa,
                 int n_steps, int step_base, int trace, cudaStream_t st);
int mega_supported();
bool mega_fits(int tmax);
void mega_set_debug(unsigned long long timeout_ns, int fault);
int mega_error_flag_offset();
int mega_trace_offset();
int mega_trace_cta_offset();

}
```

Baseline: 1313.

## Stream decoder weights through a shared-memory ring with a host-computed row plan

Replaces the persistent decode megakernel's fixed per-matrix shared-memory buffers with an 11-slot TMA ring. One thread streams weight chunks for QKV, out-proj, FC1, FC2 and LM head through the ring in order, guarded by mbarriers. A host-side plan assigns row ranges, bias offsets and attention ranks per CTA, so grids that did not fit the old row-split constraints (such as H100's SM count) can run, with an explicit co-residency check. The API also caps the megakernel at a key limit and falls back to the per-step path beyond it. The cost is more barrier waits, producer serialisation and added index arithmetic in the GEMV inner loop.

After: 1342 (median of 6 runs). +2.2%, better.

```diff
diff --git a/include/meshanything_b200.h b/include/meshanything_b200.h
--- a/include/meshanything_b200.h
+++ b/include/meshanything_b200.h
@@ -96,6 +96,8 @@
 int ma_decoder_debug(void* ws, int B, int tmax, int what, void* host_out, int nbytes);
 void ma_mega_set_debug(unsigned long long timeout_ns, int fault);
 int ma_decode_persistent_supported(void);
+#define MA_PERSISTENT_PLAN_HEAD 16
+int ma_decode_persistent_plan(int n_sm, int vocab, int n_layers, int32_t* out, int n_out);
 
 
 int ma_linear_tc_f16(const void* W, const void* bias, const void* x, int ldx, void* y, int ldy, int M, int N, int K,
diff --git a/meshanything_b200/capi.py b/meshanything_b200/capi.py
--- a/meshanything_b200/capi.py
+++ b/meshanything_b200/capi.py
@@ -40,6 +40,7 @@
     "ma_decode_slots_init", "ma_decode_slot_prefill", "ma_decode_slots_step", "ma_decode_slots_poll",
     "ma_mega_set_debug", "ma_linear_ws_set_mode", "ma_decode_slots_seek", "ma_decode_slot_stream", "ma_linear_ws_scratch_bytes", "ma_linear_ws_f16",
     "ma_sample_surface_workspace_bytes", "ma_sample_surface", "ma_tensor_core_linear_counts", "ma_decode_persistent_supported",
+    "ma_decode_persistent_plan",
 ]
 
 
@@ -94,6 +95,8 @@
     L.ma_mega_set_debug.restype = None
     L.ma_decode_persistent_supported.argtypes = []
     L.ma_decode_persistent_supported.restype = C.c_int
+    L.ma_decode_persistent_plan.argtypes = [C.c_int, C.c_int, C.c_int, _vp, C.c_int]
+    L.ma_decode_persistent_plan.restype = C.c_int
     L.ma_encoder_workspace_bytes.argtypes = [C.c_int]
     L.ma_encoder_workspace_bytes.restype = C.c_size_t
     L.ma_encoder_forward.argtypes = [_vp, _vp, C.c_int, _vp, _vp, _vp, _vp]
diff --git a/meshanything_b200/csrc/api.cu b/meshanything_b200/csrc/api.cu
--- a/meshanything_b200/csrc/api.cu
+++ b/meshanything_b200/csrc/api.cu
@@ -400,14 +400,19 @@
   const unsigned long long whash = use_graph ? weights_hash(w) : 0;
   bool flag_pending = false;
   int rc = 0;
+  int i0 = 1;
   if (mega) {
-    const int MEGA_STEPS = 512;
-    for (int i = 1; i < max_new && rc == 0; i += MEGA_STEPS) {
-      rc = mega_enqueue(w, ws.s, tmax, (__half*)kv, ws.mega, sa, std::min(MEGA_STEPS, max_new - i), i - 1,
+    const int MEGA_STEPS = 512, MEGA_MAX_KEYS = 2048;
+    const int mega_end = std::min(max_new, MEGA_MAX_KEYS - PREFIX + 1);
+    SampleArgs sm = sa;
+    sm.nkeys_next = fast_nkeys_ptr(ws.fast);
+    for (int i = 1; i < mega_end && rc == 0; i += MEGA_STEPS) {
+      rc = mega_enqueue(w, ws.s, tmax, (__half*)kv, ws.mega, sm, std::min(MEGA_STEPS, mega_end - i), i - 1,
                         (flags & MA_GEN_TRACE) ? 1 : 0, st);
     }
-  }
-  for (int i = 1; i < max_new && rc == 0 && !mega; i++) {
+    i0 = std::max(1, mega_end);
+  }
+  for (int i = i0; i < max_new && rc == 0; i++) {
     const int ctx = PREFIX + i;
     const int bucket = fast ? 0 : (ctx + 1023) / 1024;
     const int max_keys = fast ? tmax : std::min(tmax, bucket * 1024);
@@ -596,6 +601,9 @@
 
 void ma_mega_set_debug(unsigned long long timeout_ns, int fault) { mega_set_debug(timeout_ns, fault); }
 int ma_decode_persistent_supported(void) { return mega_supported(); }
+int ma_decode_persistent_plan(int n_sm, int vocab, int n_layers, int32_t* out, int n_out) {
+  return mega_plan_query(n_sm, vocab, n_layers, out, n_out);
+}
 
 int ma_decoder_debug(void* ws_, int B, int tmax, int what, void* host_out, int nbytes) {
   DecWs ws = carve(ws_, B, tmax, 8195 + 61);
diff --git a/meshanything_b200/csrc/decode_mega.cu b/meshanything_b200/csrc/decode_mega.cu
--- a/meshanything_b200/csrc/decode_mega.cu
+++ b/meshanything_b200/csrc/decode_mega.cu
@@ -1,3 +1,7 @@
+#include <algorithm>
+#include <cstring>
+#include <vector>
+
 #include "canon.cuh"
 #include "internal.h"
 
@@ -8,6 +12,23 @@
 constexpr int TEAM = 256;
 constexpr int PARTF = 66;
 constexpr int MAX_CHUNKS = 72;
+constexpr int MERGE_BLK = 31;
+
+constexpr int RING_SLOT = 16384;
+constexpr int RING_NS = 11;
+constexpr int SMEM_LIMIT = 232448;
+constexpr int MAX_CTAS = 160;
+constexpr int STAGE_MAX = 128;
+constexpr int BIAS_SLOTS = 128;
+enum { M_QKV = 0, M_OUT, M_FC1, M_FC2, M_LM, NMAT };
+
+struct MegaPlan {
+  int grid;
+  int smem;
+  int bias_off[4];
+  int row0[NMAT][MAX_CTAS + 1];
+  int arank[MAX_CTAS];
+};
 
 struct MegaWs {
   uint2 qkv_w[QKV / 2];
@@ -19,13 +40,12 @@
   int error;
   int pad_[3];
   unsigned long long trace[1280];
-  unsigned long long trace_cta[160 * 8];
+  unsigned long long trace_cta[MAX_CTAS * 8];
   ma_decoder_weights w;
+  MegaPlan plan;
   alignas(256) uint2 part_w[NHEAD * MAX_CHUNKS * PARTF];
-  alignas(256) __half bias_cta[MA_MAX_LAYERS * 160 * 128];
+  alignas(256) __half bias_cta[MA_MAX_LAYERS * MAX_CTAS * BIAS_SLOTS];
 };
-
-constexpr int BIAS_QKV = 0, BIAS_OUT = 32, BIAS_FC1 = 48, BIAS_FC2 = 112;
 
 struct MegaArgs {
   MegaWs* ws;
@@ -33,7 +53,6 @@
   __half* kv;
   long T;
   int n_steps, step_base, max_new, eos_id, pad_id;
-  int rows_qkv, rows_out, rows_fc1, rows_fc2, rows_lm;
   int32_t* out_ids;
   const int32_t* forced;
   __half* logits_out;
@@ -134,7 +153,7 @@
 }
 
 struct alignas(128) MegaSmem {
-  uint64_t bar[4];
+  uint64_t ring_bar[RING_NS];
   uint64_t lnbar[2];
   uint64_t bbar[2];
   alignas(16) float ln1[2 * HID];
@@ -148,7 +167,12 @@
   float bval[MG_WARPS];
   int bidx[MG_WARPS];
   float cstage[2 * 2 * MAX_CHUNKS];
-  alignas(16) __half stage16[64];
+  int r0[NMAT], nr[NMAT], nch[NMAT];
+  int boff[4];
+  int arank;
+  int pm, pl, pc, pj;
+  alignas(16) __half stage16[STAGE_MAX];
+  alignas(16) float mst[MERGE_BLK * PARTF];
   alignas(16) float hres[HID];
   alignas(16) __half xs[FFN];
 };
@@ -188,67 +212,72 @@
 }
 
 template <int K, bool RELU>
-__device__ __forceinline__ void gemv_stage(const __half* sw, int nrows, const __half* bias, const __half* xs, int warp,
-                                           int lane, __half* stage) {
+__device__ __forceinline__ void gemv_stage(const __half* ring, int s0, int nrows, const __half* bias, const __half* xs,
+                                           int warp, int lane, __half* stage) {
   constexpr int G = K / 256;
-  if (warp >= nrows) return;
-  const __half* w[4];
-  bool has[4];
-#pragma unroll
-  for (int i = 0; i < 4; i++) {
-    const int r = warp + MG_WARPS * i;
-    has[i] = r < nrows;
-    w[i] = sw + (size_t)(has[i] ? r : warp) * K + 8 * lane;
-  }
-  float acc[4] = {0.0f, 0.0f, 0.0f, 0.0f};
-  if (!has[1]) {
-#pragma unroll 4
-    for (int g = 0; g < G; g++) {
-      float xf[8], f[8];
-      unpack8(*reinterpret_cast<const uint4*>(xs + 256 * g + 8 * lane), xf);
-      unpack8(*reinterpret_cast<const uint4*>(w[0] + 256 * g), f);
-#pragma unroll
-      for (int j = 0; j < 8; j++) acc[0] = ffma(f[j], xf[j], acc[0]);
-    }
-  } else if (!has[2]) {
-#pragma unroll 4
-    for (int g = 0; g < G; g++) {
-      float xf[8], f0[8], f1[8];
-      unpack8(*reinterpret_cast<const uint4*>(xs + 256 * g + 8 * lane), xf);
-      unpack8(*reinterpret_cast<const uint4*>(w[0] + 256 * g), f0);
-      unpack8(*reinterpret_cast<const uint4*>(w[1] + 256 * g), f1);
-#pragma unroll
-      for (int j = 0; j < 8; j++) {
-        acc[0] = ffma(f0[j], xf[j], acc[0]);
-        acc[1] = ffma(f1[j], xf[j], acc[1]);
-      }
-    }
-  } else {
-#pragma unroll 2
-    for (int g = 0; g < G; g++) {
-      float xf[8], f[4][8];
-      unpack8(*reinterpret_cast<const uint4*>(xs + 256 * g + 8 * lane), xf);
-#pragma unroll
-      for (int i = 0; i < 4; i++) unpack8(*reinterpret_cast<const uint4*>(w[i] + 256 * g), f[i]);
-#pragma unroll
-      for (int j = 0; j < 8; j++) {
-#pragma unroll
-        for (int i = 0; i < 4; i++) acc[i] = ffma(f[i][j], xf[j], acc[i]);
-      }
-    }
-  }
-#pragma unroll
-  for (int i = 0; i < 4; i++) {
-    if (i == 0 || has[1]) acc[i] = warp_sum(acc[i]);
-  }
-  if (lane == 0) {
+  constexpr int RPS = RING_SLOT / (2 * K);
+  for (int rb = 0; rb + warp < nrows; rb += 4 * MG_WARPS) {
+    const __half* w[4];
+    bool has[4];
 #pragma unroll
     for (int i = 0; i < 4; i++) {
-      if (has[i]) {
-        const int r = warp + MG_WARPS * i;
-        __half h = __float2half_rn(fadd(acc[i], bias ? __half2float(bias[r]) : 0.0f));
-        if (RELU && __half2float(h) < 0.0f) h = __float2half_rn(0.0f);
-        stage[r] = h;
+      const int r = rb + warp + MG_WARPS * i;
+      has[i] = r < nrows;
+      const int rr = has[i] ? r : rb + warp;
+      int s = s0 + rr / RPS;
+      if (s >= RING_NS) s -= RING_NS;
+      w[i] = ring + (size_t)s * (RING_SLOT / 2) + (size_t)(rr % RPS) * K + 8 * lane;
+    }
+    float acc[4] = {0.0f, 0.0f, 0.0f, 0.0f};
+    if (!has[1]) {
+#pragma unroll 1
+      for (int g = 0; g < G; g++) {
+        float xf[8], f[8];
+        unpack8(*reinterpret_cast<const uint4*>(xs + 256 * g + 8 * lane), xf);
+        unpack8(*reinterpret_cast<const uint4*>(w[0] + 256 * g), f);
+#pragma unroll
+        for (int j = 0; j < 8; j++) acc[0] = ffma(f[j], xf[j], acc[0]);
+      }
+    } else if (!has[2]) {
+#pragma unroll 1
+      for (int g = 0; g < G; g++) {
+        float xf[8], f0[8], f1[8];
+        unpack8(*reinterpret_cast<const uint4*>(xs + 256 * g + 8 * lane), xf);
+        unpack8(*reinterpret_cast<const uint4*>(w[0] + 256 * g), f0);
+        unpack8(*reinterpret_cast<const uint4*>(w[1] + 256 * g), f1);
+#pragma unroll
+        for (int j = 0; j < 8; j++) {
+          acc[0] = ffma(f0[j], xf[j], acc[0]);
+          acc[1] = ffma(f1[j], xf[j], acc[1]);
+        }
+      }
+    } else {
+#pragma unroll 1
+      for (int g = 0; g < G; g++) {
+        float xf[8], f[4][8];
+        unpack8(*reinterpret_cast<const uint4*>(xs + 256 * g + 8 * lane), xf);
+#pragma unroll
+        for (int i = 0; i < 4; i++) unpack8(*reinterpret_cast<const uint4*>(w[i] + 256 * g), f[i]);
+#pragma unroll
+        for (int j = 0; j < 8; j++) {
+#pragma unroll
+          for (int i = 0; i < 4; i++) acc[i] = ffma(f[i][j], xf[j], acc[i]);
+        }
+      }
+    }
+#pragma unroll
+    for (int i = 0; i < 4; i++) {
+      if (i == 0 || has[1]) acc[i] = warp_sum(acc[i]);
+    }
+    if (lane == 0) {
+#pragma unroll
+      for (int i = 0; i < 4; i++) {
+        if (has[i]) {
+          const int r = rb + warp + MG_WARPS * i;
+          __half h = __float2half_rn(fadd(acc[i], bias ? __half2float(bias[r]) : 0.0f));
+          if (RELU && __half2float(h) < 0.0f) h = __float2half_rn(0.0f);
+          stage[r] = h;
+        }
       }
     }
   }
@@ -258,15 +287,31 @@
   return (uint32_t)__half_as_ushort(a) | ((uint32_t)__half_as_ushort(b) << 16);
 }
 
-__device__ __forceinline__ void refill(__half* dst, const void* W, int row0, int nrows, int K, uint64_t* bar) {
+__device__ __noinline__ void ring_produce(MegaSmem& sm, __half* ring, int n, int NL) {
+  const ma_decoder_weights& W = sm.wtab;
+  int m = sm.pm, L = sm.pl, c = sm.pc, j = sm.pj;
   fence_proxy_async();
-  if (nrows > 0) {
-    const uint32_t bytes = (uint32_t)nrows * K * 2;
-    mbar_expect_tx(bar, bytes);
-    bulk_g2s(dst, reinterpret_cast<const __half*>(W) + (size_t)row0 * K, bytes, bar);
-  } else {
-    mbar_expect_tx(bar, 0);
-  }
+  for (int k = 0; k < n; k++, j++) {
+    const int K = (m == M_FC2) ? FFN : HID, rps = RING_SLOT / (2 * K);
+    const int r = c * rps, rows = min(rps, sm.nr[m] - r);
+    const void* src = m == M_QKV ? W.wqkv[L] : m == M_OUT ? W.wo[L] : m == M_FC1 ? W.w1[L] : m == M_FC2 ? W.w2[L]
+                                                                                                      : W.lm_head;
+    const int s = j % RING_NS;
+    const uint32_t bytes = (uint32_t)rows * K * 2;
+    mbar_expect_tx(&sm.ring_bar[s], bytes);
+    bulk_g2s(ring + (size_t)s * (RING_SLOT / 2), reinterpret_cast<const __half*>(src) + (size_t)(sm.r0[m] + r) * K,
+             bytes, &sm.ring_bar[s]);
+    if (++c == sm.nch[m]) {
+      c = 0;
+      if (m == M_LM) { m = M_QKV; L = 0; }
+      else if (m == M_FC2) { if (++L == NL) m = M_LM; else m = M_QKV; }
+      else m++;
+    }
+  }
+  sm.pm = m; sm.pl = L; sm.pc = c; sm.pj = j;
+}
+__device__ __forceinline__ void ring_wait(MegaSmem& sm, int j, int n) {
+  for (int k = 0; k < n; k++, j++) mbar_wait(&sm.ring_bar[j % RING_NS], (uint32_t)(j / RING_NS) & 1u);
 }
 
 __device__ __forceinline__ void fill_ln(float* dst, const float* g, const float* b, uint64_t* bar) {
@@ -284,10 +329,7 @@
 __global__ void __launch_bounds__(MG_THREADS, 1) decode_mega_kernel(MegaArgs a) {
   extern __shared__ __align__(128) unsigned char smem_raw[];
   MegaSmem& sm = *reinterpret_cast<MegaSmem*>(smem_raw);
-  __half* bufD = reinterpret_cast<__half*>(smem_raw + sizeof(MegaSmem));
-  __half* bufC = bufD + (size_t)a.rows_qkv * HID;
-  __half* bufA = bufC + (size_t)a.rows_out * HID;
-  __half* bufB = bufA + (size_t)a.rows_fc1 * HID;
+  __half* ring = reinterpret_cast<__half*>(smem_raw + sizeof(MegaSmem));
   const int tid = threadIdx.x, warp = tid >> 5, lane = tid & 31;
   const int team = warp >> 3, wt = warp & 7, tl = tid & (TEAM - 1);
   const int grp = lane >> 3, li = lane & 7;
@@ -297,7 +339,20 @@
     uint32_t* dst = reinterpret_cast<uint32_t*>(&sm.wtab);
     for (int i = tid; i < (int)(sizeof(ma_decoder_weights) / 4); i += MG_THREADS) dst[i] = src[i];
   }
-  if (tid == 0) sm.errflag = *reinterpret_cast<volatile int*>(&ws->error);
+  const int cta = blockIdx.x, ncta = gridDim.x;
+  if (tid < NMAT) {
+    const int r0 = ws->plan.row0[tid][cta], n = ws->plan.row0[tid][cta + 1] - r0;
+    const int rps = RING_SLOT / (2 * (tid == M_FC2 ? FFN : HID));
+    sm.r0[tid] = r0;
+    sm.nr[tid] = n;
+    sm.nch[tid] = (n + rps - 1) / rps;
+    if (tid < 4) sm.boff[tid] = ws->plan.bias_off[tid];
+  }
+  if (tid == 0) {
+    sm.errflag = *reinterpret_cast<volatile int*>(&ws->error);
+    sm.arank = ws->plan.arank[cta];
+    sm.pm = M_QKV; sm.pl = 0; sm.pc = 0; sm.pj = 0;
+  }
   __syncthreads();
   if (sm.errflag) return;
   const ma_decoder_weights& W = sm.wtab;
@@ -305,31 +360,24 @@
   const long T = a.T;
   int* err = &ws->error;
 
-  const int cta = blockIdx.x, ncta = gridDim.x;
-  const int row0_qkv = cta * a.rows_qkv, n_qkv = max(0, min(a.rows_qkv, QKV - row0_qkv));
-  const int row0_out = cta * a.rows_out, n_out = max(0, min(a.rows_out, HID - row0_out));
-  const int row0_fc1 = cta * a.rows_fc1, n_fc1 = max(0, min(a.rows_fc1, FFN - row0_fc1));
-  const int row0_fc2 = cta * a.rows_fc2, n_fc2 = max(0, min(a.rows_fc2, HID - row0_fc2));
-  const int row0_lm = cta * a.rows_lm, n_lm = max(0, min(a.rows_lm, W.vocab - row0_lm));
-  const int lmD = min(n_lm, a.rows_qkv), lmC = max(0, min(n_lm, a.rows_qkv + a.rows_out) - a.rows_qkv),
-            lmA = max(0, n_lm - a.rows_qkv - a.rows_out);
-
-  uint32_t parD = 0, parC = 0, parA = 0, parB = 0, parL1 = 0, parL2 = 0, parB0 = 0, parB1 = 0;
+  uint32_t parL1 = 0, parL2 = 0, parB0 = 0, parB1 = 0;
   int lc = 0;
+  int cj = 0;
   if (tid == 0) {
-    for (int i = 0; i < 4; i++) mbar_init(&sm.bar[i], 1);
+    for (int i = 0; i < RING_NS; i++) mbar_init(&sm.ring_bar[i], 1);
     for (int i = 0; i < 2; i++) { mbar_init(&sm.lnbar[i], 1); mbar_init(&sm.bbar[i], 1); }
     mbar_fence_init();
     fill_ln(sm.ln1, W.ln1g[0], W.ln1b[0], &sm.lnbar[0]);
     fill_ln(sm.ln2, W.ln2g[0], W.ln2b[0], &sm.lnbar[1]);
-    fill_bias(sm.bias[0], ws->bias_cta + ((size_t)0 * 160 + cta) * 128, &sm.bbar[0]);
-    fill_bias(sm.bias[1], ws->bias_cta + ((size_t)(NL > 1 ? 1 : 0) * 160 + cta) * 128, &sm.bbar[1]);
-    refill(bufD, W.wqkv[0], row0_qkv, n_qkv, HID, &sm.bar[0]);
-    refill(bufC, W.wo[0], row0_out, n_out, HID, &sm.bar[1]);
-    refill(bufA, W.w1[0], row0_fc1, n_fc1, HID, &sm.bar[2]);
-    refill(bufB, W.w2[0], row0_fc2, n_fc2, FFN, &sm.bar[3]);
+    fill_bias(sm.bias[0], ws->bias_cta + ((size_t)0 * MAX_CTAS + cta) * BIAS_SLOTS, &sm.bbar[0]);
+    fill_bias(sm.bias[1], ws->bias_cta + ((size_t)(NL > 1 ? 1 : 0) * MAX_CTAS + cta) * BIAS_SLOTS, &sm.bbar[1]);
+    ring_produce(sm, ring, RING_NS, NL);
   }
   __syncthreads();
+  auto ring_release = [&](int n) {
+    if (tid == 0) ring_produce(sm, ring, n, NL);
+    cj += n;
+  };
 
   int pos = a.s.pos[0], gen = a.s.gen[0], tok = a.s.tok[0], fin = a.s.finished[0];
   unsigned long long* tr = (a.trace && cta == 0 && tid == 0) ? ws->trace : nullptr;
@@ -374,8 +422,9 @@
       __half* kc = a.kv + ((size_t)(L * 2 + 0)) * NHEAD * T * HD;
       __half* vc = a.kv + ((size_t)(L * 2 + 1)) * NHEAD * T * HD;
 
+      CSTAMP(7);
       uint4 kreg[8], vreg[8];
-      int item = team * ncta + (ncta - 1 - cta);
+      int item = team * ncta + sm.arank;
       if (item < nitems) {
         const int c = item >> 4, h = item & 15;
         const long base = ((long)h * T + (long)c * MA_ATTN_CHUNK) * HD;
@@ -430,15 +479,14 @@
       CSTAMP(0);
       mbar_wait(&sm.bbar[bsel], bsel ? parB1 : parB0);
       if (bsel) parB1 ^= 1; else parB0 ^= 1;
-      mbar_wait(&sm.bar[0], parD);
-      parD ^= 1;
+      ring_wait(sm, cj, sm.nch[M_QKV]);
       STAMP();
-      gemv_stage<HID, false>(bufD, n_qkv, lb + BIAS_QKV, sm.xs, warp, lane, sm.stage16);
+      gemv_stage<HID, false>(ring, cj % RING_NS, sm.nr[M_QKV], lb + sm.boff[M_QKV], sm.xs, warp, lane, sm.stage16);
       STAMP();
       __syncthreads();
       STAMP();
-      if (tid < (n_qkv >> 1)) {
-        const int n = row0_qkv + 2 * tid;
+      if (tid < (sm.nr[M_QKV] >> 1)) {
+        const int n = sm.r0[M_QKV] + 2 * tid;
         const uint32_t d = *reinterpret_cast<const uint32_t*>(sm.stage16 + 2 * tid);
         ll_store(ws->qkv_w + (n >> 1), d, ep);
         if (n >= HID) {
@@ -447,10 +495,7 @@
           *reinterpret_cast<uint32_t*>(c + ((long)head * T + pos) * HD + dd) = d;
         }
       }
-      if (tid == 0) {
-        if (L + 1 < NL) refill(bufD, W.wqkv[L + 1], row0_qkv, n_qkv, HID, &sm.bar[0]);
-        else refill(bufD, W.lm_head, row0_lm, lmD, HID, &sm.bar[0]);
-      }
+      ring_release(sm.nch[M_QKV]);
       STAMP();
       CSTAMP(1);
 
@@ -562,7 +607,7 @@
         const int Ln = (L + 1 < NL) ? L + 1 : 0;
         const __half* kn = a.kv + ((size_t)(Ln * 2 + 0)) * NHEAD * T * HD;
         const __half* vn = a.kv + ((size_t)(Ln * 2 + 1)) * NHEAD * T * HD;
-        for (int it2 = team * ncta + (ncta - 1 - cta); it2 < nitems; it2 += 2 * ncta) {
+        for (int it2 = team * ncta + sm.arank; it2 < nitems; it2 += 2 * ncta) {
           const int c2 = it2 >> 4, h2 = it2 & 15;
           const uint32_t bytes = (uint32_t)min(MA_ATTN_CHUNK, nkeys - c2 * MA_ATTN_CHUNK) * HD * 2;
           const long off = ((long)h2 * T + (long)c2 * MA_ATTN_CHUNK) * HD;
@@ -572,13 +617,13 @@
       }
       STAMP();
       CSTAMP(2);
-      if (team == 0 && ncta - 1 - cta < NHEAD) {
-        const int h = ncta - 1 - cta;
+      if (team == 0 && sm.arank < NHEAD) {
+        const int h = sm.arank;
         const uint2* part = ws->part_w + (long)h * MAX_CHUNKS * PARTF;
-        float* ost = reinterpret_cast<float*>(sm.xs);
+        float* ost = sm.mst;
         float* wgt = sm.cstage + team * 2 * MAX_CHUNKS;
         float* mst = wgt + MAX_CHUNKS;
-        const bool single = nch <= 31;
+        const bool single = nch <= MERGE_BLK;
         team_sync(team);
         if (!single) {
           for (int i = tl; i < nch; i += TEAM) mst[i] = __uint_as_float(ll_wait1(part + (long)i * PARTF + 64, ep, err));
@@ -588,8 +633,8 @@
           for (int i = tl; i < nch; i += TEAM) wgt[i] = ma_exp(fsub(mst[i], M));
         }
         float Lsum = 0.0f, O = 0.0f;
-        for (int c0 = 0; c0 < nch; c0 += 31) {
-          const int nb = min(31, nch - c0), nw = nb * PARTF;
+        for (int c0 = 0; c0 < nch; c0 += MERGE_BLK) {
+          const int nb = min(MERGE_BLK, nch - c0), nw = nb * PARTF;
           {
             uint2 w[8];
 #pragma unroll
@@ -642,24 +687,17 @@
       STAMP();
       CSTAMP(3);
 
-      if (n_out > 0) {
+      {
         ll_gather(ws->attn_w, HID, ep, sm.xs, err);
         __syncthreads();
-        mbar_wait(&sm.bar[1], parC);
-        gemv_stage<HID, false>(bufC, n_out, lb + BIAS_OUT, sm.xs, warp, lane, sm.stage16);
+        ring_wait(sm, cj, sm.nch[M_OUT]);
+        gemv_stage<HID, false>(ring, cj % RING_NS, sm.nr[M_OUT], lb + sm.boff[M_OUT], sm.xs, warp, lane, sm.stage16);
         __syncthreads();
         const bool withhold = a.fault && cta == a.fault - 1 && a.step_base + step >= 2;
-        if (tid < (n_out >> 1) && !withhold)
-          ll_store(ws->ya_w + ((row0_out + 2 * tid) >> 1), *reinterpret_cast<const uint32_t*>(sm.stage16 + 2 * tid), ep);
-      } else {
-        __syncthreads();
-        mbar_wait(&sm.bar[1], parC);
-      }
-      parC ^= 1;
-      if (tid == 0) {
-        if (L + 1 < NL) refill(bufC, W.wo[L + 1], row0_out, n_out, HID, &sm.bar[1]);
-        else refill(bufC, W.lm_head, row0_lm + a.rows_qkv, lmC, HID, &sm.bar[1]);
-      }
+        if (tid < (sm.nr[M_OUT] >> 1) && !withhold)
+          ll_store(ws->ya_w + ((sm.r0[M_OUT] + 2 * tid) >> 1), *reinterpret_cast<const uint32_t*>(sm.stage16 + 2 * tid), ep);
+      }
+      ring_release(sm.nch[M_OUT]);
       STAMP();
       CSTAMP(4);
 
@@ -673,35 +711,27 @@
       }
       __syncthreads();
       if (tid == 0) fill_ln(sm.ln1, W.ln1g[(L + 1) % NL], W.ln1b[(L + 1) % NL], &sm.lnbar[0]);
-      mbar_wait(&sm.bar[2], parA);
-      parA ^= 1;
-      gemv_stage<HID, true>(bufA, n_fc1, lb + BIAS_FC1, sm.xs, warp, lane, sm.stage16);
+      ring_wait(sm, cj, sm.nch[M_FC1]);
+      gemv_stage<HID, true>(ring, cj % RING_NS, sm.nr[M_FC1], lb + sm.boff[M_FC1], sm.xs, warp, lane, sm.stage16);
       __syncthreads();
-      if (tid < (n_fc1 >> 1))
-        ll_store(ws->f_w + ((row0_fc1 + 2 * tid) >> 1), *reinterpret_cast<const uint32_t*>(sm.stage16 + 2 * tid), ep);
-      if (tid == 0) {
-        if (L + 1 < NL) refill(bufA, W.w1[L + 1], row0_fc1, n_fc1, HID, &sm.bar[2]);
-        else refill(bufA, W.lm_head, row0_lm + a.rows_qkv + a.rows_out, lmA, HID, &sm.bar[2]);
-      }
+      if (tid < (sm.nr[M_FC1] >> 1))
+        ll_store(ws->f_w + ((sm.r0[M_FC1] + 2 * tid) >> 1), *reinterpret_cast<const uint32_t*>(sm.stage16 + 2 * tid), ep);
+      ring_release(sm.nch[M_FC1]);
       STAMP();
       CSTAMP(5);
 
-      if (n_fc2 > 0) {
+      {
         ll_gather(ws->f_w, FFN, ep, sm.xs, err);
         __syncthreads();
-        mbar_wait(&sm.bar[3], parB);
-        gemv_stage<FFN, false>(bufB, n_fc2, lb + BIAS_FC2, sm.xs, warp, lane, sm.stage16);
+        ring_wait(sm, cj, sm.nch[M_FC2]);
+        gemv_stage<FFN, false>(ring, cj % RING_NS, sm.nr[M_FC2], lb + sm.boff[M_FC2], sm.xs, warp, lane, sm.stage16);
         __syncthreads();
-        if (tid < (n_fc2 >> 1))
-          ll_store(ws->yb_w + ((row0_fc2 + 2 * tid) >> 1), *reinterpret_cast<const uint32_t*>(sm.stage16 + 2 * tid), ep);
-      } else {
-        __syncthreads();
-        mbar_wait(&sm.bar[3], parB);
-      }
-      parB ^= 1;
+        if (tid < (sm.nr[M_FC2] >> 1))
+          ll_store(ws->yb_w + ((sm.r0[M_FC2] + 2 * tid) >> 1), *reinterpret_cast<const uint32_t*>(sm.stage16 + 2 * tid), ep);
+      }
+      ring_release(sm.nch[M_FC2]);
       if (tid == 0) {
-        refill(bufB, W.w2[(L + 1 < NL) ? L + 1 : 0], row0_fc2, n_fc2, FFN, &sm.bar[3]);
-        fill_bias(sm.bias[bsel], ws->bias_cta + ((size_t)((L + 2) % NL) * 160 + cta) * 128, &sm.bbar[bsel]);
+        fill_bias(sm.bias[bsel], ws->bias_cta + ((size_t)((L + 2) % NL) * MAX_CTAS + cta) * BIAS_SLOTS, &sm.bbar[bsel]);
       }
       lc++;
       STAMP();
@@ -719,40 +749,35 @@
     }
     __syncthreads();
     if (tid == 0) fill_ln(sm.ln2, W.ln2g[0], W.ln2b[0], &sm.lnbar[1]);
-    mbar_wait(&sm.bar[0], parD);
-    mbar_wait(&sm.bar[1], parC);
-    mbar_wait(&sm.bar[2], parA);
-    parD ^= 1; parC ^= 1; parA ^= 1;
-    gemv_stage<HID, false>(bufD, n_lm, nullptr, sm.xs, warp, lane, sm.stage16);
+    ring_wait(sm, cj, sm.nch[M_LM]);
+    gemv_stage<HID, false>(ring, cj % RING_NS, sm.nr[M_LM], nullptr, sm.xs, warp, lane, sm.stage16);
     __syncthreads();
+    ring_release(sm.nch[M_LM]);
     float bestv = -INFINITY;
     int besti = 0x7fffffff;
-    if (tid < n_lm) {
+    if (tid < sm.nr[M_LM]) {
       const __half hv = sm.stage16[tid];
-      if (a.logits_out) a.logits_out[(long)gen * W.vocab + row0_lm + tid] = hv;
+      const int row = sm.r0[M_LM] + tid;
+      if (a.logits_out) a.logits_out[(long)gen * W.vocab + row] = hv;
       bestv = __half2float(hv);
-      besti = row0_lm + tid;
-    }
-    if (warp < 2) {
-#pragma unroll
-      for (int o = 16; o > 0; o >>= 1) {
-        const float ov = __shfl_xor_sync(0xffffffffu, bestv, o);
-        const int oi = __shfl_xor_sync(0xffffffffu, besti, o);
-        if (ov > bestv || (ov == bestv && oi < besti)) { bestv = ov; besti = oi; }
-      }
-      if (lane == 0) { sm.bval[warp] = bestv; sm.bidx[warp] = besti; }
-    }
+      besti = row;
+    }
+#pragma unroll
+    for (int o = 16; o > 0; o >>= 1) {
+      const float ov = __shfl_xor_sync(0xffffffffu, bestv, o);
+      const int oi = __shfl_xor_sync(0xffffffffu, besti, o);
+      if (ov > bestv || (ov == bestv && oi < besti)) { bestv = ov; besti = oi; }
+    }
+    if (lane == 0) { sm.bval[warp] = bestv; sm.bidx[warp] = besti; }
     __syncthreads();
     if (tid == 0) {
       float bv = sm.bval[0];
       int bi = sm.bidx[0];
-      if (sm.bval[1] > bv || (sm.bval[1] == bv && sm.bidx[1] < bi)) { bv = sm.bval[1]; bi = sm.bidx[1]; }
+      for (int w2 = 1; w2 < MG_WARPS; w2++)
+        if (sm.bval[w2] > bv || (sm.bval[w2] == bv && sm.bidx[w2] < bi)) { bv = sm.bval[w2]; bi = sm.bidx[w2]; }
       __threadfence();
       ll_store(ws->cand_w + 2 * cta, __float_as_uint(bv), epc);
       ll_store(ws->cand_w + 2 * cta + 1, (uint32_t)bi, epc);
-      refill(bufD, W.wqkv[0], row0_qkv, n_qkv, HID, &sm.bar[0]);
-      refill(bufC, W.wo[0], row0_out, n_out, HID, &sm.bar[1]);
-      refill(bufA, W.w1[0], row0_fc1, n_fc1, HID, &sm.bar[2]);
     }
     {
       float bv = -INFINITY;
@@ -793,10 +818,7 @@
     STAMP();
   }
 
-  mbar_wait(&sm.bar[0], parD);
-  mbar_wait(&sm.bar[1], parC);
-  mbar_wait(&sm.bar[2], parA);
-  mbar_wait(&sm.bar[3], parB);
+  ring_wait(sm, cj, RING_NS);
   mbar_wait(&sm.lnbar[0], parL1);
   mbar_wait(&sm.lnbar[1], parL2);
   mbar_wait(&sm.bbar[0], parB0);
@@ -818,42 +840,131 @@
     int dev = 0;
     cudaGetDevice(&dev);
     cudaDeviceGetAttribute(&g_mega_sms, cudaDevAttrMultiProcessorCount, dev);
-    if (g_mega_sms <= 0 || g_mega_sms > 160) g_mega_sms = 132;
-  }
-  return g_mega_sms;
-}
-static inline int mega_rpc(int N) { return (((N + mega_sms() - 1) / mega_sms()) + 1) & ~1; }
-
-__global__ void mega_pack_bias_kernel(MegaWs* ws, int rq, int ro, int r1, int r2) {
+    if (g_mega_sms <= 0) g_mega_sms = 132;
+  }
+  return std::min(g_mega_sms, MAX_CTAS);
+}
+
+static bool mega_make_plan(int grid, int vocab, int n_layers, MegaPlan& p, const char** why) {
+  memset(&p, 0, sizeof(p));
+  p.grid = grid;
+  p.smem = (int)(sizeof(MegaSmem) + (size_t)RING_NS * RING_SLOT);
+  *why = nullptr;
+  if (grid < NHEAD || grid > MAX_CTAS || vocab < 2 || n_layers < 1) {
+    *why = "grid out of range";
+    return false;
+  }
+  const int N[NMAT] = {QKV, HID, FFN, HID, vocab};
+  const int Kof[NMAT] = {HID, HID, HID, FFN, HID};
+  const int order[NMAT] = {M_FC2, M_FC1, M_QKV, M_OUT, M_LM};
+  long long load[MAX_CTAS] = {};
+  int cnt[NMAT][MAX_CTAS] = {};
+  for (int oi = 0; oi < NMAT; oi++) {
+    const int m = order[oi];
+    const long long pair_bytes = 2LL * 2 * Kof[m] * (m == M_LM ? 1 : n_layers);
+    const int pairs = (N[m] + 1) / 2, base = pairs / grid, extra = pairs % grid;
+    int idx[MAX_CTAS];
+    for (int c = 0; c < grid; c++) idx[c] = c;
+    std::stable_sort(idx, idx + grid, [&](int x, int y) { return load[x] < load[y]; });
+    for (int k = 0; k < grid; k++) {
+      const int c = idx[k], np = base + (k < extra ? 1 : 0);
+      cnt[m][c] = 2 * np;
+      load[c] += np * pair_bytes;
+    }
+    int r = 0;
+    for (int c = 0; c <= grid; c++) {
+      p.row0[m][c] = std::min(r, N[m]);
+      if (c < grid) r += cnt[m][c];
+    }
+  }
+  int idx[MAX_CTAS];
+  for (int c = 0; c < grid; c++) idx[c] = c;
+  std::stable_sort(idx, idx + grid, [&](int x, int y) { return load[x] < load[y] || (load[x] == load[y] && x > y); });
+  for (int k = 0; k < grid; k++) p.arank[idx[k]] = k;
+  int off = 0;
+  for (int m = 0; m < NMAT; m++) {
+    int mx = 0, mn = 1 << 30;
+    for (int c = 0; c < grid; c++) {
+      const int n = p.row0[m][c + 1] - p.row0[m][c];
+      mx = std::max(mx, n);
+      mn = std::min(mn, n);
+    }
+    if (mn < 1) *why = "a CTA owns no rows of a matrix";
+    if (mx > STAGE_MAX) *why = "too many rows of a matrix per CTA";
+    if ((mx + RING_SLOT / (2 * Kof[m]) - 1) / (RING_SLOT / (2 * Kof[m])) > RING_NS) *why = "a phase needs more than the ring";
+    if (m < 4) {
+      p.bias_off[m] = off;
+      off += mx;
+    }
+  }
+  if (off > BIAS_SLOTS) *why = "packed biases exceed their slots";
+  if (p.smem > SMEM_LIMIT) *why = "shared memory";
+  return *why == nullptr;
+}
+
+static const MegaPlan* mega_plan(int grid, int vocab, int n_layers, const char** why) {
+  struct Entry { int grid, vocab, nl; bool ok; const char* why; MegaPlan p; };
+  static std::vector<Entry*> cache;
+  for (Entry* e : cache)
+    if (e->grid == grid && e->vocab == vocab && e->nl == n_layers) {
+      *why = e->why;
+      return e->ok ? &e->p : nullptr;
+    }
+  Entry* e = new Entry;
+  e->grid = grid; e->vocab = vocab; e->nl = n_layers;
+  e->ok = mega_make_plan(grid, vocab, n_layers, e->p, &e->why);
+  cache.push_back(e);
+  *why = e->why;
+  return e->ok ? &e->p : nullptr;
+}
+
+int mega_plan_query(int n_sm, int vocab, int n_layers, int32_t* out, int n_out) {
+  if (n_sm < 1 || n_sm > MAX_CTAS || !out || n_out < MA_PERSISTENT_PLAN_HEAD + 6 * n_sm + 5) return -1;
+  MegaPlan p;
+  const char* why;
+  const bool ok = mega_make_plan(n_sm, vocab, n_layers, p, &why);
+  memset(out, 0, sizeof(int32_t) * n_out);
+  out[0] = p.grid;
+  out[1] = p.smem;
+  out[2] = RING_NS;
+  out[3] = RING_SLOT;
+  for (int m = 0; m < 4; m++) out[4 + m] = p.bias_off[m];
+  out[8] = BIAS_SLOTS;
+  out[9] = (int)sizeof(MegaSmem);
+  int32_t* o = out + MA_PERSISTENT_PLAN_HEAD;
+  for (int m = 0; m < NMAT; m++)
+    for (int c = 0; c <= n_sm; c++) *o++ = p.row0[m][c];
+  for (int c = 0; c < n_sm; c++) *o++ = p.arank[c];
+  return ok ? 1 : 0;
+}
+
+__global__ void mega_pack_bias_kernel(MegaWs* ws) {
   const int L = blockIdx.y, cta = blockIdx.x, t = threadIdx.x;
   const ma_decoder_weights& W = ws->w;
+  const MegaPlan& p = ws->plan;
   __half v = __float2half_rn(0.0f);
-  if (t < BIAS_OUT) {
-    const int n = cta * rq + t;
-    if (t < rq && n < QKV) v = reinterpret_cast<const __half*>(W.bqkv[L])[n];
-  } else if (t < BIAS_FC1) {
-    const int i = t - BIAS_OUT, n = cta * ro + i;
-    if (i < ro && n < HID) v = reinterpret_cast<const __half*>(W.bo[L])[n];
-  } else if (t < BIAS_FC2) {
-    const int i = t - BIAS_FC1, n = cta * r1 + i;
-    if (i < r1 && n < FFN) v = reinterpret_cast<const __half*>(W.b1[L])[n];
-  } else {
-    const int i = t - BIAS_FC2, n = cta * r2 + i;
-    if (i < r2 && n < HID) v = reinterpret_cast<const __half*>(W.b2[L])[n];
-  }
-  ws->bias_cta[((size_t)L * 160 + cta) * 128 + t] = v;
+  if (cta < p.grid) {
+    const void* b[4] = {W.bqkv[L], W.bo[L], W.b1[L], W.b2[L]};
+    for (int m = 0; m < 4; m++) {
+      const int i = t - p.bias_off[m], r0 = p.row0[m][cta];
+      if (i >= 0 && i < p.row0[m][cta + 1] - r0) v = reinterpret_cast<const __half*>(b[m])[r0 + i];
+    }
+  }
+  ws->bias_cta[((size_t)L * MAX_CTAS + cta) * BIAS_SLOTS + t] = v;
 }
 
 int mega_prepare(const ma_decoder_weights* w, void* mega_ws, cudaStream_t st) {
   MegaWs* ws = reinterpret_cast<MegaWs*>(mega_ws);
+  const char* why;
+  const MegaPlan* p = mega_plan(mega_sms(), w->vocab, w->n_layers, &why);
+  if (!p) {
+    set_error("mega: no row plan for %d SMs: %s", mega_sms(), why);
+    return 1;
+  }
   if (cudaMemsetAsync(ws, 0, offsetof(MegaWs, bias_cta), st) != cudaSuccess) return 1;
   if (cudaMemcpyAsync(&ws->w, w, sizeof(ma_decoder_weights), cudaMemcpyHostToDevice, st) != cudaSuccess) return 1;
-  const int rq = mega_rpc(QKV), ro = mega_rpc(HID), r1 = mega_rpc(FFN), r2 = mega_rpc(HID);
-  if (rq > 32 || ro > 16 || r1 > 64 || r2 > 16) {
-    set_error("mega: rows per CTA out of range");
-    return 1;
-  }
-  mega_pack_bias_kernel<<<dim3(160, w->n_layers), 128, 0, st>>>(ws, rq, ro, r1, r2);
+  if (cudaMemcpyAsync(&ws->plan, p, sizeof(MegaPlan), cudaMemcpyHostToDevice, st) != cudaSuccess) return 1;
+  mega_pack_bias_kernel<<<dim3(MAX_CTAS, w->n_layers), BIAS_SLOTS, 0, st>>>(ws);
   count_launch();
   return check_launch("mega_pack_bias_kernel") ? 0 : 1;
 }
@@ -868,13 +979,39 @@
   g_mega_fault = fault;
 }
 bool mega_fits(int tmax) { return tmax <= MAX_CHUNKS * MA_ATTN_CHUNK; }
+static bool mega_residency_ok(int smem, int grid) {
+  static int attr_set = 0;
+  if (smem > attr_set) {
+    if (cudaFuncSetAttribute(decode_mega_kernel, cudaFuncAttributeMaxDynamicSharedMemorySize, smem) != cudaSuccess) {
+      set_error("mega: cannot get %d bytes of shared memory", smem);
+      cudaGetLastError();
+      return false;
+    }
+    attr_set = smem;
+  }
+  int per_sm = 0;
+  if (cudaOccupancyMaxActiveBlocksPerMultiprocessor(&per_sm, decode_mega_kernel, MG_THREADS, smem) != cudaSuccess) {
+    cudaGetLastError();
+    per_sm = 0;
+  }
+  int dev = 0, sms = 0;
+  cudaGetDevice(&dev);
+  cudaDeviceGetAttribute(&sms, cudaDevAttrMultiProcessorCount, dev);
+  if (per_sm < 1 || grid > per_sm * sms) {
+    set_error("mega: %d CTAs of %d threads and %d bytes of shared memory are not co-resident (%d per SM, %d SMs)", grid,
+              MG_THREADS, smem, per_sm, sms);
+    return false;
+  }
+  return true;
+}
+
 int mega_supported() {
   static int ok = -1;
   if (ok < 0) {
-    const int sms = mega_sms(), r1 = mega_rpc(FFN), ro = mega_rpc(HID);
-    const int grid = (FFN + r1 - 1) / r1;
-    ok = (grid <= sms && grid >= NHEAD && grid - NHEAD >= (HID + ro - 1) / ro && mega_rpc(QKV) <= 32 && ro <= 16 && r1 <= 64) ? 1 : 0;
-    if (!ok) set_error("mega: unsupported SM count %d", sms);
+    const char* why;
+    const MegaPlan* p = mega_plan(mega_sms(), 8195, 24, &why);
+    if (!p) set_error("mega: no row plan for %d SMs: %s", mega_sms(), why);
+    ok = (p && mega_residency_ok(p->smem, p->grid)) ? 1 : 0;
   }
   return ok;
 }
@@ -888,8 +1025,13 @@
     set_error("mega: tmax=%d exceeds %d keys", tmax, MAX_CHUNKS * MA_ATTN_CHUNK);
     return 1;
   }
-  const int sms = mega_sms();
-  auto rpc = [&](int N) { return mega_rpc(N); };
+  const char* why;
+  const MegaPlan* p = mega_plan(mega_sms(), w->vocab, w->n_layers, &why);
+  if (!p) {
+    set_error("mega: no row plan for %d SMs: %s", mega_sms(), why);
+    return 1;
+  }
+  if (!mega_residency_ok(p->smem, p->grid)) return 1;
   MegaArgs a;
   memset(&a, 0, sizeof(a));
   a.ws = reinterpret_cast<MegaWs*>(mega_ws);
@@ -899,38 +1041,14 @@
   a.n_steps = n_steps;
   a.step_base = step_base;
   a.max_new = sa.max_new; a.eos_id = sa.eos_id; a.pad_id = sa.pad_id;
-  a.rows_qkv = rpc(QKV); a.rows_out = rpc(HID); a.rows_fc1 = rpc(FFN); a.rows_fc2 = rpc(HID); a.rows_lm = rpc(w->vocab);
   a.out_ids = sa.out_ids; a.forced = sa.forced; a.logits_out = sa.logits_out; a.all_done = sa.all_done;
   a.nkeys_next = sa.nkeys_next;
   a.trace = trace;
   a.fault = g_mega_fault;
-  if (a.rows_lm > a.rows_qkv + a.rows_out + a.rows_fc1 || a.rows_lm > 64 || a.rows_fc1 > 64) {
-    set_error("mega: rows per CTA out of range (lm %d, fc1 %d)", a.rows_lm, a.rows_fc1);
-    return 1;
-  }
-  const int grid = (FFN + a.rows_fc1 - 1) / a.rows_fc1;
-  if (grid > sms || (w->vocab + a.rows_lm - 1) / a.rows_lm != grid || grid < NHEAD) {
-    set_error("mega: unsupported SM count %d (grid %d)", sms, grid);
-    return 1;
-  }
-  if (grid - NHEAD < (HID + a.rows_out - 1) / a.rows_out) {
-    set_error("mega: the last %d CTAs must not own out_proj rows (grid %d)", NHEAD, grid);
-    return 1;
-  }
-  const size_t smem = sizeof(MegaSmem) + ((size_t)(a.rows_qkv + a.rows_out + a.rows_fc1) * HID + (size_t)a.rows_fc2 * FFN) * 2;
-  static size_t attr_set = 0;
-  if (smem > attr_set) {
-    if (cudaFuncSetAttribute(decode_mega_kernel, cudaFuncAttributeMaxDynamicSharedMemorySize, (int)smem) != cudaSuccess) {
-      set_error("mega: cannot get %zu bytes of shared memory", smem);
-      cudaGetLastError();
-      return 1;
-    }
-    attr_set = smem;
-  }
   cudaLaunchConfig_t cfg = {};
-  cfg.gridDim = dim3(grid);
+  cfg.gridDim = dim3(p->grid);
   cfg.blockDim = dim3(MG_THREADS);
-  cfg.dynamicSmemBytes = smem;
+  cfg.dynamicSmemBytes = p->smem;
   cfg.stream = st;
   cudaLaunchAttribute at[1];
   at[0].id = cudaLaunchAttributeCooperative;
diff --git a/meshanything_b200/csrc/internal.h b/meshanything_b200/csrc/internal.h
--- a/meshanything_b200/csrc/internal.h
+++ b/meshanything_b200/csrc/internal.h
@@ -96,6 +96,7 @@
 int mega_enqueue(const ma_decoder_weights* w, SeqState s, int tmax, __half* kv, void* mega_ws, const SampleArgs& sa,
                  int n_steps, int step_base, int trace, cudaStream_t st);
 int mega_supported();
+int mega_plan_query(int n_sm, int vocab, int n_layers, int32_t* out, int n_out);
 bool mega_fits(int tmax);
 void mega_set_debug(unsigned long long timeout_ns, int fault);
 int mega_error_flag_offset();
```
